# PimLb/POMDP_PBVI_Exploration

Hardware: AMD Instinct MI355X
Metric: alpha-vector backups/sec (higher is better)
Workload: dtype f32

## Files before the change

### include/pbvi_hip.h

```cpp
#ifndef PBVI_HIP_H
#define PBVI_HIP_H

#include <stddef.h>
#include <stdint.h>

#ifdef __cplusplus
extern "C" {
#endif

typedef struct pbvi_engine pbvi_engine_t;

enum pbvi_status {
    PBVI_OK = 0,
    PBVI_EINVAL = -1,
    PBVI_ENOMEM = -2,
    PBVI_ERUNTIME = -3,
    PBVI_EUNSUPPORTED = -4
};

enum pbvi_dtype { PBVI_F32 = 0, PBVI_F64 = 1 };

enum pbvi_mode {
    PBVI_SPARSE = 0,
    PBVI_DENSE = 1
};

enum pbvi_flags {
    PBVI_BELIEF_DOMINANCE = 1
};

typedef struct pbvi_stats {
    double ms_total;
    double ms_project;
    double ms_score;
    double ms_argmax;
    double ms_refine;
    double ms_action;
    double ms_assemble;
    double ms_dominance;
    int64_t n_pairs;
    int64_t n_dead;
    int64_t n_refined;
    int64_t n_refined_actions;
    int64_t n_unique;
    int64_t score_flops;
    int64_t score_flops_executed;
    int64_t score_tiles_dense;
    int64_t score_tiles_run;
    int64_t project_flops;
    int64_t project_flops_executed;
    int32_t split_k;
    int32_t formulation;
    int64_t n_refine_candidates;
    double ms_project_gemm;
    int32_t screened;
    int32_t fused_projection;
    int32_t score_split;
    int32_t gamma_chunks;
} pbvi_stats_t;

int pbvi_version(void);
int pbvi_device_count(void);
const char* pbvi_last_error(void);

int pbvi_engine_create(pbvi_engine_t** out, int device, int32_t S, int32_t A, int32_t O, int32_t R,
                       const int32_t* reach_states, const void* rto, const void* exp_reward,
                       int dtype, int mode);
void pbvi_engine_destroy(pbvi_engine_t* e);

int pbvi_alpha_set(pbvi_engine_t* e, const void* alpha, int64_t V);
int pbvi_alpha_append(pbvi_engine_t* e, const void* alpha, int64_t V_add);
int64_t pbvi_alpha_count(const pbvi_engine_t* e);

int pbvi_beliefs_set(pbvi_engine_t* e, const void* beliefs, int64_t B);

int64_t pbvi_alpha_store_append(pbvi_engine_t* e, const void* rows , int64_t n);
int pbvi_alpha_select(pbvi_engine_t* e, const int32_t* ids , int64_t V);
int pbvi_alpha_layout(pbvi_engine_t* e, int64_t* free_rows, int64_t* layouts);
int pbvi_alpha_store_reset(pbvi_engine_t* e);
int64_t pbvi_belief_store_append(pbvi_engine_t* e, const void* rows , int64_t n);
int pbvi_beliefs_select(pbvi_engine_t* e, const int32_t* ids , int64_t B);
int pbvi_belief_store_reset(pbvi_engine_t* e);

int pbvi_backup_run(pbvi_engine_t* e, double gamma, int flags, pbvi_stats_t* stats );

int pbvi_backup_fetch(pbvi_engine_t* e, void* out_alpha, int32_t* out_action,
                      int32_t* out_best_alpha, uint8_t* out_keep);

int64_t pbvi_backup_unique_count(const pbvi_engine_t* e);
int pbvi_backup_fetch_unique(pbvi_engine_t* e, void* out_rows, int32_t* out_index);

int pbvi_backup_fetch_compact(pbvi_engine_t* e, void* out_rows, int32_t* out_index, int32_t* out_action,
                              int32_t* out_best_alpha, uint8_t* out_keep);

int pbvi_backup_run_fetch(pbvi_engine_t* e, double gamma, int flags, pbvi_stats_t* stats, void* out_rows, int64_t cap_rows,
                          int32_t* out_slot, int32_t* out_index, int32_t* out_action, int32_t* out_best_alpha, uint8_t* out_keep,
                          int64_t* n_unique, int64_t* n_slots);

int pbvi_backup_fetch_row_hashes(pbvi_engine_t* e, uint64_t* out_hashes);

void* pbvi_host_alloc(size_t bytes);
void pbvi_host_free(void* p);

int64_t pbvi_backup_store_unique(pbvi_engine_t* e, const int32_t* unique_idx, int64_t n);

int pbvi_backup_fetch_unique_keys(pbvi_engine_t* e, int32_t* out_keys);
int pbvi_backup_fetch_exchange(pbvi_engine_t* e, int32_t* out);
int pbvi_backup_fetch_exchange_padded(pbvi_engine_t* e, int64_t per, int32_t* out);
int pbvi_assemble_rows(pbvi_engine_t* e, double gamma, int64_t n, const int32_t* keys, void* out_rows);
int64_t pbvi_assemble_rows_store(pbvi_engine_t* e, double gamma, int64_t n, const int32_t* keys, void* out_rows);
int64_t pbvi_exchange_merge(const int32_t* all_meta, int32_t world, int64_t stride, int64_t per, int32_t key_width,
                            int64_t n_total, int32_t* out_keys, int32_t* out_index, int32_t* out_action, uint8_t* out_keep);

int pbvi_backup_device_results(pbvi_engine_t* e, void** d_alpha, int32_t** d_action, uint8_t** d_keep);

int pbvi_backup(pbvi_engine_t* e, const void* beliefs, int64_t B, double gamma, int flags,
                void* out_alpha, int32_t* out_action, int32_t* out_best_alpha, uint8_t* out_keep,
                pbvi_stats_t* stats);

int pbvi_prune_dominated(pbvi_engine_t* e, uint8_t* keep );

int pbvi_value_max(pbvi_engine_t* e, double* out_value, int32_t* out_index);

int pbvi_value_max_store(pbvi_engine_t* e, int64_t n, double* out_value, int32_t* out_index);
int pbvi_backup_fetch_value_max(pbvi_engine_t* e, double* out_value);
int64_t pbvi_belief_store_count(const pbvi_engine_t* e);
int64_t pbvi_alpha_store_count(const pbvi_engine_t* e);

int pbvi_set_value_max_exact(pbvi_engine_t* e, int exact);

int pbvi_belief_update(pbvi_engine_t* e, const int32_t* actions, const int32_t* observations, void* out_beliefs);

int pbvi_beliefs_advance(pbvi_engine_t* e, const int32_t* actions, const int32_t* observations, const uint8_t* keep,
                         int64_t* out_B);
int pbvi_beliefs_fetch(pbvi_engine_t* e, void* out_beliefs);
int64_t pbvi_beliefs_count(const pbvi_engine_t* e);

int pbvi_mdp_value_iteration(int device, int32_t S, int32_t A, int32_t R, const int32_t* reach_states,
                             const double* reach_prob, const double* exp_reward, const double* v0, double gamma,
                             double max_change_limit, int32_t horizon, double* out_rows, double* out_changes,
                             int32_t* out_iterations);

int64_t pbvi_belief_walk(pbvi_engine_t* e, const double* b0, int64_t n, const int32_t* actions, const int32_t* observations,
                         const uint8_t* restart, double* out_beliefs);
int pbvi_belief_walk_keys(pbvi_engine_t* e, int64_t n, uint64_t* out_keys);
int pbvi_engine_set_rto_f64(pbvi_engine_t* e, const double* rto);

int pbvi_set_formulation(pbvi_engine_t* e, int formulation);

int pbvi_set_f64_screen(pbvi_engine_t* e, int mode);

int pbvi_set_fused_projection(pbvi_engine_t* e, int enable);

int pbvi_set_score_split(pbvi_engine_t* e, int mode);

int pbvi_set_gamma_tiling(pbvi_engine_t* e, int mode, int64_t chunk_rows);
int pbvi_gamma_tiling_plan(int32_t S, int32_t A, int32_t O, int64_t V, int64_t B, int dtype, int64_t budget_bytes,
                           int64_t* chunk_rows, int64_t* n_chunks, int64_t* bytes_needed);

int pbvi_set_tie_window(pbvi_engine_t* e, double rel);

int pbvi_debug_poison(int enable);
int64_t pbvi_debug_alloc_limit(int64_t mb);
int pbvi_engine_after_oom(pbvi_engine_t* e);

int pbvi_debug_gemm_dense(int enable);

int64_t pbvi_device_bytes(const pbvi_engine_t* e);

#ifdef __cplusplus
}
#endif
#endif
```

### pomdp_pbvi_exploration_amd/csrc/engine.hip

```cpp
#include <algorithm>
#include <cmath>
#include <cstdio>
#include <cstdlib>
#include <cstring>
#include <condition_variable>
#include <mutex>
#include <new>
#include <string>
#include <thread>
#include <unistd.h>
#include <vector>

#include "backup_kernels.h"
#include "split_bf16.h"

namespace pbvi {

static thread_local std::string g_err;
static int g_poison = -1;
static bool poison_enabled() {
    if (g_poison < 0) g_poison = getenv("PBVI_POISON") != nullptr ? 1 : 0;
    return g_poison == 1;
}
void set_error(const std::string& msg) { g_err = msg; }
// ... 3523 lines not shown
    do {                                                   \
        if (!(e) || !(e)->impl) {                          \
            pbvi::set_error("NULL engine handle");         \
            return PBVI_EINVAL;                            \
        }                                                  \
    } while (0)

int pbvi_alpha_set(pbvi_engine_t* e, const void* alpha, int64_t V) {
    NEED(e);
    return e->impl->alpha_set(alpha, V);
}
int pbvi_alpha_append(pbvi_engine_t* e, const void* alpha, int64_t V_add) {
    NEED(e);
    return e->impl->alpha_append(alpha, V_add);
}
int64_t pbvi_alpha_count(const pbvi_engine_t* e) { return (e && e->impl) ? e->impl->alpha_count() : -1; }
int pbvi_beliefs_set(pbvi_engine_t* e, const void* beliefs, int64_t B) {
    NEED(e);
    return e->impl->beliefs_set(beliefs, B);
}
int pbvi_backup_run(pbvi_engine_t* e, double gamma, int flags, pbvi_stats_t* stats) {
    NEED(e);
    return e->impl->backup_run(gamma, flags, stats);
}
int pbvi_backup_fetch(pbvi_engine_t* e, void* out_alpha, int32_t* out_action, int32_t* out_best_alpha, uint8_t* out_keep) {
    NEED(e);
    return e->impl->backup_fetch(out_alpha, out_action, out_best_alpha, out_keep);
}
int64_t pbvi_backup_store_unique(pbvi_engine_t* e, const int32_t* unique_idx, int64_t n) {
    NEED(e);
    return e->impl->store_append_unique(unique_idx, n);
}

int pbvi_backup_fetch_row_hashes(pbvi_engine_t* e, uint64_t* out_hashes) {
    NEED(e);
    return e->impl->fetch_row_hashes(out_hashes);
}
int pbvi_backup_fetch_unique_keys(pbvi_engine_t* e, int32_t* out_keys) {
    NEED(e);
    return e->impl->fetch_unique_keys(out_keys);
}
int pbvi_backup_fetch_exchange(pbvi_engine_t* e, int32_t* out) {
    NEED(e);
    return e->impl->fetch_exchange(out, e->impl->beliefs_count());
}
int pbvi_backup_fetch_exchange_padded(pbvi_engine_t* e, int64_t per, int32_t* out) {
    NEED(e);
    return e->impl->fetch_exchange(out, per);
}
int64_t pbvi_assemble_rows_store(pbvi_engine_t* e, double gamma, int64_t n, const int32_t* keys, void* out_rows) {
    NEED(e);
    return e->impl->assemble_keys_store(gamma, n, keys, out_rows);
}
int64_t pbvi_exchange_merge(const int32_t* all_meta, int32_t world, int64_t stride, int64_t per, int32_t key_width,
                            int64_t n_total, int32_t* out_keys, int32_t* out_index, int32_t* out_action, uint8_t* out_keep) {
    if (!all_meta || world <= 0 || per <= 0 || key_width <= 0 || n_total < 0 || !out_keys || !out_index ||
        !out_action || !out_keep) {
        pbvi::set_error("exchange_merge: bad arguments");
        return PBVI_EINVAL;
    }
    const int64_t n_meta = 1 + 3 * per + per * (int64_t)key_width;
    if (per > 0x7fffffff / ((int64_t)key_width + 3) || stride < n_meta || n_total > (int64_t)world * per ||
        (int64_t)world * per > 0x7fffffff) {
        pbvi::set_error("exchange_merge: message stride / belief count do not fit the block size");
        return PBVI_EINVAL;
    }
    int64_t total = 0;
    for (int r = 0; r < world; ++r) {
        const int64_t c = all_meta[(int64_t)r * stride];
        if (c < 0 || c > per) {
            pbvi::set_error("exchange_merge: corrupt message (unique-row count out of range)");
            return PBVI_EINVAL;
        }
        total += c;
    }
    size_t cap = 16;
    while (cap < (size_t)total * 2 + 1) cap <<= 1;
    std::vector<int32_t> table, pos;
    try {
        table.assign(cap, -1);
        pos.assign((size_t)std::max<int64_t>(total, 1), 0);
    } catch (const std::bad_alloc&) {
        pbvi::set_error("exchange_merge: host allocation failed");
        return PBVI_ENOMEM;
    }
    int64_t n_keys = 0, base = 0;
    for (int r = 0; r < world; ++r) {
        const int32_t* msg = all_meta + (int64_t)r * stride;
        const int32_t* keys = msg + 1 + 3 * per;
        const int64_t c = msg[0];
        for (int64_t u = 0; u < c; ++u) {
            const int32_t* k = keys + u * key_width;
            uint64_t h = 1469598103934665603ull;
            for (int j = 0; j < key_width; ++j) h = (h ^ (uint32_t)k[j]) * 1099511628211ull;
            size_t slot = (size_t)(h ^ (h >> 29)) & (cap - 1);
            for (;;) {
                const int32_t at = table[slot];
                if (at < 0) {
                    std::memcpy(out_keys + n_keys * key_width, k, (size_t)key_width * sizeof(int32_t));
                    table[slot] = (int32_t)n_keys;
                    pos[(size_t)(base + u)] = (int32_t)n_keys++;
                    break;
                }
                if (std::memcmp(out_keys + (int64_t)at * key_width, k, (size_t)key_width * sizeof(int32_t)) == 0) {
                    pos[(size_t)(base + u)] = at;
                    break;
                }
                slot = (slot + 1) & (cap - 1);
            }
        }
        const int64_t lo = std::min<int64_t>((int64_t)r * per, n_total), hi = std::min<int64_t>(lo + per, n_total);
        for (int64_t j = 0; j < hi - lo; ++j) {
            const int32_t u = msg[1 + j];
            if (u < 0 || u >= c) {
                pbvi::set_error("exchange_merge: corrupt message (row index out of range)");
                return PBVI_EINVAL;
            }
            out_index[lo + j] = pos[(size_t)(base + u)];
            out_action[lo + j] = msg[1 + per + j];
            out_keep[lo + j] = msg[1 + 2 * per + j] ? 1 : 0;
        }
        base += c;
    }
    return n_keys;
}
int pbvi_assemble_rows(pbvi_engine_t* e, double gamma, int64_t n, const int32_t* keys, void* out_rows) {
    NEED(e);
    return e->impl->assemble_keys(gamma, n, keys, out_rows);
}
int pbvi_engine_after_oom(pbvi_engine_t* e) {
    NEED(e);
    return e->impl->after_oom();
}
int pbvi_backup_device_results(pbvi_engine_t* e, void** d_alpha, int32_t** d_action, uint8_t** d_keep) {
    NEED(e);
    return e->impl->device_results(d_alpha, d_action, d_keep);
}
int64_t pbvi_backup_unique_count(const pbvi_engine_t* e) { return (e && e->impl) ? e->impl->unique_count() : -1; }
int pbvi_backup_fetch_unique(pbvi_engine_t* e, void* out_rows, int32_t* out_index) {
    NEED(e);
    return e->impl->fetch_unique(out_rows, out_index);
}
int pbvi_backup_run_fetch(pbvi_engine_t* e, double gamma, int flags, pbvi_stats_t* stats, void* out_rows, int64_t cap_rows,
                          int32_t* out_slot, int32_t* out_index, int32_t* out_action, int32_t* out_best_alpha, uint8_t* out_keep,
                          int64_t* n_unique, int64_t* n_slots) {
    NEED(e);
    return e->impl->run_fetch(gamma, flags, stats, out_rows, cap_rows, out_slot, out_index, out_action, out_best_alpha, out_keep,
                              n_unique, n_slots);
}
int pbvi_backup_fetch_compact(pbvi_engine_t* e, void* out_rows, int32_t* out_index, int32_t* out_action,
                              int32_t* out_best_alpha, uint8_t* out_keep) {
    NEED(e);
    return e->impl->fetch_compact(out_rows, out_index, out_action, out_best_alpha, out_keep);
}
void* pbvi_host_alloc(size_t bytes) {
    void* p = nullptr;
    if (bytes == 0) return nullptr;
    if (hipHostMalloc(&p, bytes, hipHostMallocDefault) != hipSuccess) {
        (void)hipGetLastError();
        pbvi::set_error("pbvi_host_alloc: hipHostMalloc of " + std::to_string(bytes) + " bytes failed");
        return nullptr;
    }
    return p;
}
void pbvi_host_free(void* p) {
    if (p && hipHostFree(p) != hipSuccess) (void)hipGetLastError();
}
int pbvi_debug_gemm_dense(int enable) { return pbvi::set_gemm_force_dense(enable); }
int pbvi_backup(pbvi_engine_t* e, const void* beliefs, int64_t B, double gamma, int flags, void* out_alpha,
                int32_t* out_action, int32_t* out_best_alpha, uint8_t* out_keep, pbvi_stats_t* stats) {
    NEED(e);
    int rc = e->impl->beliefs_set(beliefs, B);
    if (rc) return rc;
    rc = e->impl->backup_run(gamma, flags, stats);
    if (rc) return rc;
    return e->impl->backup_fetch(out_alpha, out_action, out_best_alpha, out_keep);
}
int pbvi_prune_dominated(pbvi_engine_t* e, uint8_t* keep) {
    NEED(e);
    return e->impl->prune_dominated(keep);
}
int pbvi_value_max(pbvi_engine_t* e, double* out_value, int32_t* out_index) {
    NEED(e);
    return e->impl->value_max(out_value, out_index);
}
int64_t pbvi_alpha_store_append(pbvi_engine_t* e, const void* rows, int64_t n) {
    NEED(e);
    return e->impl->store_append(0, rows, n);
}
int pbvi_value_max_store(pbvi_engine_t* e, int64_t n, double* out_value, int32_t* out_index) {
    NEED(e);
    return e->impl->value_max_store(n, out_value, out_index);
}
int64_t pbvi_belief_store_count(const pbvi_engine_t* e) { return (e && e->impl) ? e->impl->store_count(1) : -1; }
int64_t pbvi_alpha_store_count(const pbvi_engine_t* e) { return (e && e->impl) ? e->impl->store_count(0) : -1; }
int pbvi_alpha_select(pbvi_engine_t* e, const int32_t* ids, int64_t V) {
    NEED(e);
    return e->impl->store_select(0, ids, V);
}
int pbvi_alpha_store_reset(pbvi_engine_t* e) {
    NEED(e);
    return e->impl->store_reset(0);
}
int64_t pbvi_belief_store_append(pbvi_engine_t* e, const void* rows, int64_t n) {
    NEED(e);
    return e->impl->store_append(1, rows, n);
}
int pbvi_beliefs_select(pbvi_engine_t* e, const int32_t* ids, int64_t B) {
    NEED(e);
    return e->impl->store_select(1, ids, B);
}
int pbvi_belief_store_reset(pbvi_engine_t* e) {
    NEED(e);
    return e->impl->store_reset(1);
}
int pbvi_beliefs_advance(pbvi_engine_t* e, const int32_t* actions, const int32_t* observations, const uint8_t* keep,
                         int64_t* out_B) {
    NEED(e);
    return e->impl->beliefs_advance(actions, observations, keep, out_B);
}

int pbvi_backup_fetch_value_max(pbvi_engine_t* e, double* out_value) {
    NEED(e);
    return e->impl->backup_value_max(out_value);
}
int pbvi_belief_walk_keys(pbvi_engine_t* e, int64_t n, uint64_t* out_keys) {
    NEED(e);
    return e->impl->walk_keys(n, out_keys);
}
int64_t pbvi_belief_walk(pbvi_engine_t* e, const double* b0, int64_t n, const int32_t* actions, const int32_t* observations,
                         const uint8_t* restart, double* out_beliefs) {
    NEED(e);
    return e->impl->belief_walk(b0, n, actions, observations, restart, out_beliefs);
}

int pbvi_engine_set_rto_f64(pbvi_engine_t* e, const double* rto) {
    NEED(e);
    return e->impl->set_rto_f64(rto);
}

int pbvi_beliefs_fetch(pbvi_engine_t* e, void* out_beliefs) {
    NEED(e);
    return e->impl->beliefs_fetch(out_beliefs);
}

int64_t pbvi_beliefs_count(const pbvi_engine_t* e) { return (e && e->impl) ? e->impl->beliefs_count() : -1; }

int pbvi_mdp_value_iteration(int device, int32_t S, int32_t A, int32_t R, const int32_t* reach_states,
                             const double* reach_prob, const double* exp_reward, const double* v0, double gamma,
                             double max_change_limit, int32_t horizon, double* out_rows, double* out_changes,
                             int32_t* out_iterations) {
    return pbvi::mdp_value_iteration(device, S, A, R, reach_states, reach_prob, exp_reward, v0, gamma, max_change_limit,
                                     horizon, out_rows, out_changes, out_iterations);
}

int pbvi_belief_update(pbvi_engine_t* e, const int32_t* actions, const int32_t* observations, void* out_beliefs) {
    NEED(e);
    return e->impl->belief_update(actions, observations, out_beliefs);
}
int pbvi_set_formulation(pbvi_engine_t* e, int formulation) {
    NEED(e);
    return e->impl->set_formulation(formulation);
}
int pbvi_set_fused_projection(pbvi_engine_t* e, int enable) {
    NEED(e);
    return e->impl->set_fused(enable);
}
int pbvi_set_f64_screen(pbvi_engine_t* e, int mode) {
    NEED(e);
    return e->impl->set_screen(mode);
}
int pbvi_set_score_split(pbvi_engine_t* e, int mode) {
    NEED(e);
    return e->impl->set_score_split(mode);
}
int pbvi_set_value_max_exact(pbvi_engine_t* e, int exact) {
    NEED(e);
    return e->impl->set_value_max_exact(exact);
}
int pbvi_alpha_layout(pbvi_engine_t* e, int64_t* free_rows, int64_t* layouts) {
    NEED(e);
    return e->impl->alpha_layout(free_rows, layouts);
}
int pbvi_set_gamma_tiling(pbvi_engine_t* e, int mode, int64_t chunk_rows) {
    NEED(e);
    return e->impl->set_gamma_tiling(mode, chunk_rows);
}
int pbvi_gamma_tiling_plan(int32_t S, int32_t A, int32_t O, int64_t V, int64_t B, int dtype, int64_t budget_bytes,
                           int64_t* chunk_rows, int64_t* n_chunks, int64_t* bytes_needed) {
    using namespace pbvi;
    if (!chunk_rows || !n_chunks || !bytes_needed || (dtype != 0 && dtype != 1))
        FAIL(PBVI_EINVAL, "gamma_tiling_plan: null output or dtype not 0 (fp32) / 1 (fp64)");
    pbvi::TilingPlan tp;
    const int rc = pbvi::tiling_plan(S, A, O, V, B, dtype == 0, budget_bytes, *chunk_rows, &tp);
    if (rc == PBVI_EINVAL) FAIL(PBVI_EINVAL, "gamma_tiling_plan: S, A, O, V, B must be positive, budget and chunk_rows >= 0, A*O*(V+1)+2A within int32");
    *chunk_rows = tp.chunk_rows;
    *n_chunks = tp.n_chunks;
    *bytes_needed = tp.bytes;
    if (rc == PBVI_ENOMEM)
        FAIL(PBVI_ENOMEM, "gamma_tiling_plan: chunks of " + std::to_string(tp.chunk_rows) + " alpha rows need " +
                              std::to_string(tp.bytes) + " bytes, the budget is " + std::to_string(budget_bytes));
    return PBVI_OK;
}
int pbvi_set_tie_window(pbvi_engine_t* e, double rel) {
    NEED(e);
    return e->impl->set_tie_window(rel);
}
int64_t pbvi_device_bytes(const pbvi_engine_t* e) { return (e && e->impl) ? e->impl->device_bytes() : -1; }

}
```

### pomdp_pbvi_exploration_amd/csrc/gemm.hip

```cpp
#include "pbvi_common.h"
#include "split_bf16.h"

#include <cstdlib>
#include <map>
#include <mutex>

namespace pbvi {

typedef float f32x4 __attribute__((ext_vector_type(4)));
typedef float f32x16 __attribute__((ext_vector_type(16)));

constexpr int TILE_FLOATS = 256 * GEMM_BK;
constexpr int KL_IRR_BIT = 30;
constexpr int KL_MASK = (1 << KL_IRR_BIT) - 1;
constexpr int GEMM_LDS_BYTES = 4 * TILE_FLOATS * 4;

__device__ __forceinline__ void glds16(const float* g, float* l) {
    __builtin_amdgcn_global_load_lds((const __attribute__((address_space(1))) void*)g,
                                     (__attribute__((address_space(3))) void*)l, 16, 0, 0);
}

struct TileThread {
    int lane, wid, i, h, wr, wc;
    int srow[4], scol[4];
    int a_row[4], b_row[2];
    __device__ __forceinline__ void init() {
        const int tid = threadIdx.x;
        lane = tid & 63;
        wid = __builtin_amdgcn_readfirstlane(tid >> 6);
        i = lane & 31;
        h = lane >> 5;
        wr = wid >> 2;
        wc = wid & 3;
#pragma unroll
        for (int it = 0; it < 4; ++it) {
            const int c = it * 512 + tid;
            const int row = c >> 3, pc = c & 7;
            srow[it] = row;
            scol[it] = (pc ^ ((row >> 1) & 7)) * 4;
        }
#pragma unroll
        for (int mi = 0; mi < 4; ++mi) a_row[mi] = wr * 128 + mi * 32 + i;
#pragma unroll
        for (int ni = 0; ni < 2; ++ni) b_row[ni] = wc * 64 + ni * 32 + i;
    }
};

__device__ __forceinline__ void tile_stage(const TileThread& t, float* lds, int buf, const float* Ablk, int lda,
                                           const float* Bblk, int ldb, int kt) {
    float* la = lds + buf * 2 * TILE_FLOATS;
    float* lb = la + TILE_FLOATS;
#pragma unroll
    for (int it = 0; it < 4; ++it) {
        const int wave_chunk = it * 512 + t.wid * 64;
        glds16(Ablk + (int64_t)t.srow[it] * lda + kt * GEMM_BK + t.scol[it], la + wave_chunk * 4);
        glds16(Bblk + (int64_t)t.srow[it] * ldb + kt * GEMM_BK + t.scol[it], lb + wave_chunk * 4);
    }
}

__device__ __forceinline__ void tile_compute_group(const TileThread& t, const float* lds, int buf, f32x16 (&acc)[4][2], int g) {
    const float* la = lds + buf * 2 * TILE_FLOATS;
    const float* lb = la + TILE_FLOATS;
    f32x4 af[4], bf[2];
#pragma unroll
    for (int mi = 0; mi < 4; ++mi) {
        const int pc = (2 * g + t.h) ^ ((t.a_row[mi] >> 1) & 7);
        af[mi] = *(const f32x4*)(la + t.a_row[mi] * GEMM_BK + pc * 4);
    }
#pragma unroll
    for (int ni = 0; ni < 2; ++ni) {
        const int pc = (2 * g + t.h) ^ ((t.b_row[ni] >> 1) & 7);
        bf[ni] = *(const f32x4*)(lb + t.b_row[ni] * GEMM_BK + pc * 4);
    }
#pragma unroll
    for (int j = 0; j < 4; ++j)
#pragma unroll
        for (int mi = 0; mi < 4; ++mi)
#pragma unroll
            for (int ni = 0; ni < 2; ++ni)
                acc[mi][ni] = __builtin_amdgcn_mfma_f32_32x32x2f32(af[mi][j], bf[ni][j], acc[mi][ni], 0, 0, 0);
}

__device__ __forceinline__ void tile_compute(const TileThread& t, const float* lds, int buf, f32x16 (&acc)[4][2]) {
#pragma unroll
    for (int g = 0; g < 4; ++g) tile_compute_group(t, lds, buf, acc, g);
}

__device__ __forceinline__ void tile_run(const TileThread& t, float* lds, const float* Ablk, int lda, const float* Bblk,
                                         int ldb, const int* __restrict__ kl, int i0, int i1, f32x16 (&acc)[4][2]) {
    tile_stage(t, lds, 0, Ablk, lda, Bblk, ldb, kl[i0] & KL_MASK);
    int k_next = (i0 + 1 < i1) ? (kl[i0 + 1] & KL_MASK) : 0;
    asm volatile("s_waitcnt vmcnt(0)" ::: "memory");
    __syncthreads();
    int buf = 0;
    for (int it = i0; it < i1; ++it) {
        int k_after = 0;
        if (it + 1 < i1) {
            tile_stage(t, lds, buf ^ 1, Ablk, lda, Bblk, ldb, k_next);
            if (it + 2 < i1) k_after = kl[it + 2] & KL_MASK;
        }
        tile_compute(t, lds, buf, acc);
        asm volatile("s_waitcnt vmcnt(0)" ::: "memory");
        __syncthreads();
        buf ^= 1;
        k_next = k_after;
    }
}

__device__ __forceinline__ void tile_zero(f32x16 (&acc)[4][2]) {
#pragma unroll
    for (int mi = 0; mi < 4; ++mi)
#pragma unroll
        for (int ni = 0; ni < 2; ++ni)
#pragma unroll
            for (int e = 0; e < 16; ++e) acc[mi][ni][e] = 0.f;
}

__device__ __forceinline__ void tile_store(const TileThread& t, float* Cz, int ldc, int tm, int tn,
                                           const f32x16 (&acc)[4][2]) {
#pragma unroll
    for (int mi = 0; mi < 4; ++mi)
#pragma unroll
        for (int ni = 0; ni < 2; ++ni) {
            const int col = tn * 256 + t.wc * 64 + ni * 32 + t.i;
#pragma unroll
            for (int e = 0; e < 16; ++e) {
                const int row = tm * 256 + t.wr * 128 + mi * 32 + (e & 3) + 8 * (e >> 2) + 4 * t.h;
                Cz[(int64_t)row * ldc + col] = acc[mi][ni][e];
            }
        }
}

__global__ __launch_bounds__(512) void k_gemm_nt_f32_mfma(
    const float* __restrict__ A, int lda, const float* __restrict__ B, int ldb, float* __restrict__ C,
    int ldc, int64_t slab_stride, int tiles_m, int tiles_n, int k_tiles, int chunk_len, int max_chunks,
    const int* __restrict__ klist, const int* __restrict__ kcount, int64_t batch_stride_b, int64_t batch_stride_c) {
    extern __shared__ __attribute__((aligned(16))) float lds[];
    const int bid = blockIdx.x;
    const int xcd = bid & 7, slot = bid >> 3;
    const int tm = slot % tiles_m;
    const int q = (slot / tiles_m) * 8 + xcd;
    const int tn = q % tiles_n;
    const int z = q / tiles_n;
    if (z >= max_chunks) return;
    const int batch = blockIdx.y;
    B += batch * batch_stride_b;
    C += batch * batch_stride_c;
    const int pair = (batch * tiles_n + tn) * tiles_m + tm;
    const int cnt = kcount[pair];
    const int i0 = z * chunk_len;
    const int i1 = (i0 + chunk_len < cnt) ? i0 + chunk_len : cnt;
    if (i0 >= i1) return;
    TileThread t;
    t.init();
    f32x16 acc[4][2];
    tile_zero(acc);
    tile_run(t, lds, A + (int64_t)tm * 256 * lda, lda, B + (int64_t)tn * 256 * ldb, ldb,
             klist + (int64_t)pair * k_tiles, i0, i1, acc);
    tile_store(t, C + (int64_t)z * slab_stride, ldc, tm, tn, acc);
}

__global__ void k_streamk_plan(const int* __restrict__ kcount, int pairs, int nblocks, int k_tiles, int max_split,
                               int ovh, int* __restrict__ prefix, int* __restrict__ start_pair,
                               int* __restrict__ first_block, int* __restrict__ nchunks, int* __restrict__ plan) {
    __shared__ int part[256];
    __shared__ int q_sh;
    const int tid = threadIdx.x;
    const int per = (pairs + 255) / 256;
    const int p0 = (tid * per < pairs) ? tid * per : pairs;
    const int p1 = (p0 + per < pairs) ? p0 + per : pairs;
    int sum = 0;
    for (int p = p0; p < p1; ++p) {
        const int cnt = kcount[p];
        sum += cnt > 0 ? cnt + ovh : 0;
    }
    part[tid] = sum;
    for (int i = tid; i < nblocks; i += 256) start_pair[i] = -1;
    __syncthreads();
    if (tid == 0) {
        int run = 0;
        for (int i = 0; i < 256; ++i) {
            const int v = part[i];
            part[i] = run;
            run += v;
        }
        int q = (run + nblocks - 1) / nblocks;
        const int qmin = (k_tiles + ovh + max_split - 1) / max_split;
        if (q < qmin) q = qmin;
        if (q < 1) q = 1;
        q_sh = q;
        plan[0] = q;
        plan[1] = run;
        prefix[pairs] = run;
    }
    __syncthreads();
    const int q = q_sh;
    int run = part[tid];
    for (int p = p0; p < p1; ++p) {
        const int cnt = kcount[p];
        prefix[p] = run;
        if (cnt > 0) {
            const int cost = cnt + ovh;
            const int fb = run / q, lb = (run + cost - 1) / q;
            const int fw = (run + ovh) / q;
            first_block[p] = fw;
            nchunks[p] = lb - fw + 1;
            for (int i = fb; i <= lb; ++i)
                if ((int64_t)i * q >= run) start_pair[i] = p;
            run += cost;
        } else {
            first_block[p] = 0;
            nchunks[p] = 0;
        }
    }
}

__global__ __launch_bounds__(512) void k_gemm_nt_f32_streamk(
    const float* __restrict__ A, int lda, const float* __restrict__ B, int ldb, float* __restrict__ C, int ldc,
    int64_t slab_stride, int tiles_m, int pairs, int k_tiles, const int* __restrict__ klist,
    const int* __restrict__ kcount, const int* __restrict__ prefix, const int* __restrict__ start_pair,
    const int* __restrict__ first_block, const int* __restrict__ plan, int ovh) {
    extern __shared__ __attribute__((aligned(16))) float lds[];
    const int nb = gridDim.x;
    int L;
    {
        const int bid = blockIdx.x, xcd = bid & 7, qq = nb >> 3, r = nb & 7;
        const int base = (xcd < r) ? xcd * (qq + 1) : r * (qq + 1) + (xcd - r) * qq;
        L = base + (bid >> 3);
    }
    const int q = plan[0], T = plan[1];
    int64_t pos = (int64_t)L * q;
    if (pos >= T) return;
    const int64_t end = (pos + q < T) ? pos + q : T;
    int p = start_pair[L];
    if (p < 0) return;
    TileThread t;
    t.init();
    while (pos < end && p < pairs) {
        const int cnt = kcount[p];
        if (cnt == 0) {
            ++p;
            continue;
        }
        const int u_lo = (int)(pos - prefix[p]);
        const int64_t room = end - pos;
        const int u_hi = (u_lo + room < cnt + ovh) ? (int)(u_lo + room) : cnt + ovh;
        const int lo = u_lo > ovh ? u_lo - ovh : 0;
        const int hi = u_hi > ovh ? u_hi - ovh : 0;
        if (hi > lo) {
            const int tm = p % tiles_m, tn = p / tiles_m;
            f32x16 acc[4][2];
            tile_zero(acc);
            tile_run(t, lds, A + (int64_t)tm * 256 * lda, lda, B + (int64_t)tn * 256 * ldb, ldb,
                     klist + (int64_t)p * k_tiles, lo, hi, acc);
            const bool cont = L != first_block[p];
            tile_store(t, cont ? C + slab_stride + (int64_t)L * (256 * 256) : C, cont ? 256 : ldc, cont ? 0 : tm, cont ? 0 : tn, acc);
        }
        pos += u_hi - u_lo;
        ++p;
    }
}

typedef int i32x4 __attribute__((ext_vector_type(4)));
#ifndef PBVI_FUSED_EXP
#define PBVI_FUSED_EXP 0
#endif

__device__ __forceinline__ void ld16(f32x4& dst, const float* p) {
    asm volatile("global_load_dwordx4 %0, %1, off" : "=v"(dst) : "v"(p) : "memory");
}
__device__ __forceinline__ void ld16i(i32x4& dst, const int32_t* p) {
    asm volatile("global_load_dwordx4 %0, %1, off" : "=v"(dst) : "v"(p) : "memory");
}
__device__ __forceinline__ void ld4(float& dst, const float* p) {
    asm volatile("global_load_dword %0, %1, off" : "=v"(dst) : "v"(p) : "memory");
}

__device__ __forceinline__ f32x4 fused_value(float gamma, f32x4 w, f32x4 av) {
#pragma clang fp contract(off)
    const f32x4 pr = w * av;
    return gamma * pr;
}

__device__ __forceinline__ void tile_run_fused(const TileThread& t, float* lds, const float* Ablk, int lda,
                                               const int32_t* __restrict__ rsrow, const float* __restrict__ rtorow,
                                               const float* __restrict__ arow0, int64_t a_step ,
                                               float gamma, const int* __restrict__ kl,
                                               int i0, int i1, f32x16 (&acc)[4][2]) {
    const int tid = threadIdx.x;
    auto stage_a = [&](int buf, int entry) {
        const int kt = entry & KL_MASK;
        float* la = lds + buf * 2 * TILE_FLOATS;
#pragma unroll
        for (int it = 0; it < 4; ++it)
            glds16(Ablk + (int64_t)t.srow[it] * lda + kt * GEMM_BK + t.scol[it], la + (it * 512 + t.wid * 64) * 4);
    };
    i32x4 idx;
    f32x4 w, av[4];
    auto tables = [&](int entry) {
        const int s = (entry & KL_MASK) * GEMM_BK + t.scol[0];
        ld16i(idx, rsrow + s);
        ld16(w, rtorow + s);
    };
    auto alphas = [&](int entry) {
        if (entry >> KL_IRR_BIT) {
#pragma unroll
            for (int it = 0; it < 4; ++it) {
                const float* arow = arow0 + it * a_step;
                float e0, e1, e2, e3;
                ld4(e0, arow + idx[0]);
                ld4(e1, arow + idx[1]);
                ld4(e2, arow + idx[2]);
                ld4(e3, arow + idx[3]);
                asm volatile("s_waitcnt vmcnt(0)\n\tv_mov_b32 %0, %4\n\tv_mov_b32 %1, %5\n\tv_mov_b32 %2, %6\n\tv_mov_b32 %3, %7"
                             : "=&v"(av[it].x), "=&v"(av[it].y), "=&v"(av[it].z), "=&v"(av[it].w)
                             : "v"(e0), "v"(e1), "v"(e2), "v"(e3)
                             : "memory");
            }
        } else {
#if PBVI_FUSED_EXP == 1
#pragma unroll
            for (int it = 0; it < 4; ++it) av[it] = w;
#else
#pragma unroll
            for (int it = 0; it < 4; ++it) ld16(av[it], arow0 + it * a_step + idx[0]);
#endif
        }
    };
    auto store_b = [&](int buf) {
        float* lb = lds + buf * 2 * TILE_FLOATS + TILE_FLOATS;
#if PBVI_FUSED_EXP == 2
        if (gamma == 12345.f)
#endif
#pragma unroll
        for (int it = 0; it < 4; ++it) *(f32x4*)(lb + (it * 512 + tid) * 4) = fused_value(gamma, w, av[it]);
    };
    tables(kl[i0]);
    stage_a(0, kl[i0]);
    asm volatile("s_waitcnt vmcnt(0)" : "+v"(idx), "+v"(w)::"memory");
    alphas(kl[i0]);
    asm volatile("s_waitcnt vmcnt(0)" : "+v"(av[0]), "+v"(av[1]), "+v"(av[2]), "+v"(av[3])::"memory");
    store_b(0);
    int k_next = (i0 + 1 < i1) ? kl[i0 + 1] : 0;
    __syncthreads();
    int buf = 0;
    for (int it = i0; it < i1; ++it) {
        int k_after = 0;
        const bool more = it + 1 < i1;
        if (more) {
            tables(k_next);
            stage_a(buf ^ 1, k_next);
            if (it + 2 < i1) k_after = kl[it + 2];
        }
        tile_compute_group(t, lds, buf, acc, 0);
        if (more) {
            asm volatile("s_waitcnt vmcnt(4)" : "+v"(idx), "+v"(w)::"memory");
            alphas(k_next);
        }
        tile_compute_group(t, lds, buf, acc, 1);
        tile_compute_group(t, lds, buf, acc, 2);
        if (more) {
            asm volatile("s_waitcnt vmcnt(0)" : "+v"(av[0]), "+v"(av[1]), "+v"(av[2]), "+v"(av[3])::"memory");
            store_b(buf ^ 1);
        }
        tile_compute_group(t, lds, buf, acc, 3);
        asm volatile("s_waitcnt vmcnt(0)" ::: "memory");
        __syncthreads();
        buf ^= 1;
        k_next = k_after;
    }
}

__global__ __launch_bounds__(512) void k_gemm_nt_f32_streamk_fused(
    const float* __restrict__ A, int lda, const float* __restrict__ B, int ldb, FusedB fb, float* __restrict__ C, int ldc,
    int64_t slab_stride, int tiles_m, int pairs, int k_tiles, const int* __restrict__ klist, const int* __restrict__ kcount,
    const int* __restrict__ prefix, const int* __restrict__ start_pair, const int* __restrict__ first_block,
    const int* __restrict__ plan, int ovh) {
    extern __shared__ __attribute__((aligned(16))) float lds[];
    const int nb = gridDim.x;
    int L;
    {
        const int bid = blockIdx.x, xcd = bid & 7, qq = nb >> 3, r = nb & 7;
        const int base = (xcd < r) ? xcd * (qq + 1) : r * (qq + 1) + (xcd - r) * qq;
        L = base + (bid >> 3);
    }
    const int q = plan[0], T = plan[1];
    int64_t pos = (int64_t)L * q;
    if (pos >= T) return;
    const int64_t end = (pos + q < T) ? pos + q : T;
    int p = start_pair[L];
    if (p < 0) return;
    TileThread t;
    t.init();
    while (pos < end && p < pairs) {
        const int cnt = kcount[p];
        if (cnt == 0) {
            ++p;
            continue;
        }
        const int u_lo = (int)(pos - prefix[p]);
        const int64_t room = end - pos;
        const int u_hi = (u_lo + room < cnt + ovh) ? (int)(u_lo + room) : cnt + ovh;
        const int lo = u_lo > ovh ? u_lo - ovh : 0;
        const int hi = u_hi > ovh ? u_hi - ovh : 0;
        if (hi > lo) {
            const int tm = p % tiles_m, tn = p / tiles_m;
            f32x16 acc[4][2];
            tile_zero(acc);
            if (fb.mat[tn]) {
                const int bt = fb.ctile != nullptr ? fb.ctile[tn] : tn;
                tile_run(t, lds, A + (int64_t)tm * 256 * lda, lda, B + (int64_t)bt * 256 * ldb, ldb,
                         klist + (int64_t)p * k_tiles, lo, hi, acc);
            } else {
                const int r0 = tn * 256;
                const int g = r0 / fb.V, v0 = r0 - g * fb.V;
                tile_run_fused(t, lds, A + (int64_t)tm * 256 * lda, lda, fb.rs + (int64_t)(g / fb.O) * fb.S_pad,
                               fb.rto + (int64_t)g * fb.S_pad, fb.alpha + (int64_t)(v0 + t.srow[0]) * fb.lda,
                               (int64_t)64 * fb.lda, fb.gamma,
                               klist + (int64_t)p * k_tiles, lo, hi, acc);
            }
            const bool cont = L != first_block[p];
            tile_store(t, cont ? C + slab_stride + (int64_t)L * (256 * 256) : C, cont ? 256 : ldc, cont ? 0 : tm, cont ? 0 : tn, acc);
        }
        pos += u_hi - u_lo;
        ++p;
    }
}

constexpr int FUSED_R_MAX = 7;
constexpr int TAB_WORDS = 8 * GEMM_BK;
constexpr int GEMM_LDS_BYTES_R = GEMM_LDS_BYTES + 2 * 2 * TAB_WORDS * 4;

struct Frag {
    f32x4 af[4], bf[2];
};
__device__ __forceinline__ void frag_load(const TileThread& t, const float* lds, int buf, int g, Frag& f) {
    const float* la = lds + buf * 2 * TILE_FLOATS;
    const float* lb = la + TILE_FLOATS;
#pragma unroll
    for (int mi = 0; mi < 4; ++mi) {
        const int pc = (2 * g + t.h) ^ ((t.a_row[mi] >> 1) & 7);
        f.af[mi] = *(const f32x4*)(la + t.a_row[mi] * GEMM_BK + pc * 4);
    }
#pragma unroll
    for (int ni = 0; ni < 2; ++ni) {
        const int pc = (2 * g + t.h) ^ ((t.b_row[ni] >> 1) & 7);
        f.bf[ni] = *(const f32x4*)(lb + t.b_row[ni] * GEMM_BK + pc * 4);
    }
}
__device__ __forceinline__ void frag_mfma(const Frag& f, int j, f32x16 (&acc)[4][2]) {
#pragma unroll
    for (int mi = 0; mi < 4; ++mi)
#pragma unroll
        for (int ni = 0; ni < 2; ++ni)
            acc[mi][ni] = __builtin_amdgcn_mfma_f32_32x32x2f32(f.af[mi][j], f.bf[ni][j], acc[mi][ni], 0, 0, 0);
}

__device__ __forceinline__ f32x4 proj_add(f32x4 acc, f32x4 w, f32x4 av) {
#pragma clang fp contract(off)
    const f32x4 pr = w * av;
    return acc + pr;
}
__device__ __forceinline__ f32x4 proj_scale(float gamma, f32x4 acc) {
#pragma clang fp contract(off)
    return gamma * acc;
}

template <int R>
__device__ __forceinline__ void tile_run_fused_r(const TileThread& t, float* lds, const float* Ablk, int lda,
                                                 const float* Bblk, int ldb, const int32_t* __restrict__ rs_a,
                                                 const float* __restrict__ rto_g, int S_pad,
                                                 const float* __restrict__ arow0, int64_t a_step ,
                                                 float gamma, const int* __restrict__ kl, int i0, int i1,
                                                 f32x16 (&acc)[4][2]) {
    const int tid = threadIdx.x;
    int32_t* tabi = (int32_t*)(lds + 4 * TILE_FLOATS);
    float* tabw = (float*)(tabi + 2 * TAB_WORDS);
    constexpr int nunits = 2 * R;
    static_assert(R >= 2 && R <= FUSED_R_MAX, "2R + 2 issue points must fit the 16 of a K step");
    const int scol0 = t.scol[0];
    auto stage_a = [&](int buf, int entry) {
        const int kt = entry & KL_MASK;
        float* la = lds + buf * 2 * TILE_FLOATS;
#pragma unroll
        for (int it = 0; it < 4; ++it)
            glds16(Ablk + (int64_t)t.srow[it] * lda + kt * GEMM_BK + t.scol[it], la + (it * 512 + t.wid * 64) * 4);
    };
    auto stage_b = [&](int buf, int entry) {
        const int kt = entry & KL_MASK;
        float* lb = lds + buf * 2 * TILE_FLOATS + TILE_FLOATS;
#pragma unroll
        for (int it = 0; it < 4; ++it)
            glds16(Bblk + (int64_t)t.srow[it] * ldb + kt * GEMM_BK + t.scol[it], lb + (it * 512 + t.wid * 64) * 4);
    };
    auto stage_tab = [&](int tb, int entry) {
        if (t.wid == 0 && t.lane < 8 * R) {
            const int64_t off = (int64_t)(t.lane >> 3) * S_pad + (entry & KL_MASK) * GEMM_BK + (t.lane & 7) * 4;
            glds16((const float*)(rs_a + off), (float*)(tabi + tb * TAB_WORDS));
            glds16(rto_g + off, tabw + tb * TAB_WORDS);
        }
    };
    f32x4 av[2][2];
    f32x4 pacc[2];
    auto unit_issue = [&](int u, int slot, int tb) {
        const int hh = u >= R ? 1 : 0, r = u - hh * R;
        const i32x4 idx = *(const i32x4*)(tabi + tb * TAB_WORDS + r * GEMM_BK + scol0);
#if PBVI_FUSED_EXP == 3
        const float* p0 = arow0 + (int64_t)(2 * hh) * a_step + (idx[0] & 3);
#else
        const float* p0 = arow0 + (int64_t)(2 * hh) * a_step + idx[0];
#endif
        ld16(av[slot][0], p0);
        ld16(av[slot][1], p0 + a_step);
    };
    auto unit_consume = [&](int u, int slot, int tb, int dst_buf, bool last_in_queue) {
        const int hh = u >= R ? 1 : 0, r = u - hh * R;
        const f32x4 w = *(const f32x4*)(tabw + tb * TAB_WORDS + r * GEMM_BK + scol0);
        if (last_in_queue)
            asm volatile("s_waitcnt vmcnt(0)" : "+v"(av[slot][0]), "+v"(av[slot][1])::"memory");
        else
            asm volatile("s_waitcnt vmcnt(2)" : "+v"(av[slot][0]), "+v"(av[slot][1])::"memory");
        if (r == 0) {
            pacc[0] = f32x4{0.f, 0.f, 0.f, 0.f};
            pacc[1] = f32x4{0.f, 0.f, 0.f, 0.f};
        }
        pacc[0] = proj_add(pacc[0], w, av[slot][0]);
        pacc[1] = proj_add(pacc[1], w, av[slot][1]);
        if (r == R - 1) {
            float* lb = lds + dst_buf * 2 * TILE_FLOATS + TILE_FLOATS;
            *(f32x4*)(lb + ((2 * hh) * 512 + tid) * 4) = proj_scale(gamma, pacc[0]);
            *(f32x4*)(lb + ((2 * hh + 1) * 512 + tid) * 4) = proj_scale(gamma, pacc[1]);
        }
    };
    {
        const int e0 = kl[i0];
        stage_a(0, e0);
        if (e0 >> KL_IRR_BIT) {
            stage_b(0, e0);
        } else {
            stage_tab(0, e0);
            asm volatile("s_waitcnt vmcnt(0)" ::: "memory");
            __syncthreads();
            for (int u = 0; u < nunits; ++u) {
                unit_issue(u, 0, 0);
                unit_consume(u, 0, 0, 0, true);
            }
        }
    }
    int e_next = (i0 + 1 < i1) ? kl[i0 + 1] : 0;
    if (i0 + 1 < i1 && !(e_next >> KL_IRR_BIT)) stage_tab(1, e_next);
    int e_after = (i0 + 2 < i1) ? kl[i0 + 2] : 0;
    asm volatile("s_waitcnt vmcnt(0)" ::: "memory");
    __syncthreads();
    int buf = 0;
    for (int it = i0; it < i1; ++it) {
        const bool more = it + 1 < i1;
        const bool gen = more && !(e_next >> KL_IRR_BIT);
        int e_after2 = 0;
        if (more) {
            stage_a(buf ^ 1, e_next);
            if (!gen) stage_b(buf ^ 1, e_next);
            if (it + 2 < i1 && !(e_after >> KL_IRR_BIT)) stage_tab(buf, e_after);
            if (it + 3 < i1) e_after2 = kl[it + 3];
        }
        Frag f;
#pragma unroll
        for (int g = 0; g < 4; ++g) {
            frag_load(t, lds, buf, g, f);
#pragma unroll
            for (int j = 0; j < 4; ++j) {
                const int p = 4 * g + j;
                if (gen) {
                    if (p >= 2 && p - 2 < nunits) unit_consume(p - 2, p & 1, buf ^ 1, buf ^ 1, p - 2 == nunits - 1);
                    if (p < nunits) unit_issue(p, p & 1, buf ^ 1);
                }
                frag_mfma(f, j, acc);
            }
        }
        asm volatile("s_waitcnt vmcnt(0)" ::: "memory");
        __syncthreads();
        buf ^= 1;
        e_next = e_after;
        e_after = e_after2;
    }
}

template <int R>
__global__ __launch_bounds__(512) void k_gemm_nt_f32_streamk_fused_r(
    const float* __restrict__ A, int lda, const float* __restrict__ B, int ldb, FusedB fb, float* __restrict__ C, int ldc,
    int64_t slab_stride, int tiles_m, int pairs, int k_tiles, const int* __restrict__ klist, const int* __restrict__ kcount,
    const int* __restrict__ prefix, const int* __restrict__ start_pair, const int* __restrict__ first_block,
    const int* __restrict__ plan, int ovh) {
    extern __shared__ __attribute__((aligned(16))) float lds[];
    const int nb = gridDim.x;
    int L;
    {
        const int bid = blockIdx.x, xcd = bid & 7, qq = nb >> 3, r = nb & 7;
        const int base = (xcd < r) ? xcd * (qq + 1) : r * (qq + 1) + (xcd - r) * qq;
        L = base + (bid >> 3);
    }
    const int q = plan[0], T = plan[1];
    int64_t pos = (int64_t)L * q;
    if (pos >= T) return;
    const int64_t end = (pos + q < T) ? pos + q : T;
    int p = start_pair[L];
    if (p < 0) return;
    TileThread t;
    t.init();
    while (pos < end && p < pairs) {
        const int cnt = kcount[p];
        if (cnt == 0) {
            ++p;
            continue;
        }
        const int u_lo = (int)(pos - prefix[p]);
        const int64_t room = end - pos;
        const int u_hi = (u_lo + room < cnt + ovh) ? (int)(u_lo + room) : cnt + ovh;
        const int lo = u_lo > ovh ? u_lo - ovh : 0;
        const int hi = u_hi > ovh ? u_hi - ovh : 0;
        if (hi > lo) {
            const int tm = p % tiles_m, tn = p / tiles_m;
            f32x16 acc[4][2];
            tile_zero(acc);
            if (fb.mat[tn]) {
                tile_run(t, lds, A + (int64_t)tm * 256 * lda, lda, B + (int64_t)tn * 256 * ldb, ldb,
                         klist + (int64_t)p * k_tiles, lo, hi, acc);
            } else {
                const int r0 = tn * 256;
                const int g = r0 / fb.V, v0 = r0 - g * fb.V;
                tile_run_fused_r<R>(t, lds, A + (int64_t)tm * 256 * lda, lda, B + (int64_t)tn * 256 * ldb, ldb,
                                 fb.rs + (int64_t)(g / fb.O) * R * fb.S_pad, fb.rto + (int64_t)g * R * fb.S_pad,
                                 fb.S_pad, fb.alpha + (int64_t)(v0 + t.srow[0]) * fb.lda, (int64_t)64 * fb.lda, fb.gamma,
                                 klist + (int64_t)p * k_tiles, lo, hi, acc);
            }
            const bool cont = L != first_block[p];
            tile_store(t, cont ? C + slab_stride + (int64_t)L * (256 * 256) : C, cont ? 256 : ldc, cont ? 0 : tm, cont ? 0 : tn, acc);
        }
        pos += u_hi - u_lo;
        ++p;
    }
}

typedef __bf16 bf16x8 __attribute__((ext_vector_type(8)));

__device__ __forceinline__ void split_store(float* lop, int row, int kg, const f32x4& x0, const f32x4& x1) {
    i32x4 hi, lo;
    uint32_t h, l;
    split_pair(x0[0], x0[1], h, l); hi[0] = (int)h; lo[0] = (int)l;
    split_pair(x0[2], x0[3], h, l); hi[1] = (int)h; lo[1] = (int)l;
    split_pair(x1[0], x1[1], h, l); hi[2] = (int)h; lo[2] = (int)l;
    split_pair(x1[2], x1[3], h, l); hi[3] = (int)h; lo[3] = (int)l;
    const int sw = (row >> 1) & 7;
    *(i32x4*)(lop + row * GEMM_BK + (kg ^ sw) * 4) = hi;
    *(i32x4*)(lop + row * GEMM_BK + ((4 + kg) ^ sw) * 4) = lo;
}

struct SplitFrag {
    i32x4 ah[4], al[4], bh[2], bl[2];
};
__device__ __forceinline__ void split_group(const TileThread& t, const float* lds, int buf, int kk, int term, SplitFrag& f,
                                            f32x16 (&acc)[4][2]) {
    const float* la = lds + buf * 2 * TILE_FLOATS;
    const float* lb = la + TILE_FLOATS;
    const int hc = 2 * kk + t.h;
    if (term != 1) {
#pragma unroll
        for (int mi = 0; mi < 4; ++mi) {
            const int r = t.a_row[mi], sw = (r >> 1) & 7;
            if (term == 0) f.ah[mi] = *(const i32x4*)(la + r * GEMM_BK + (hc ^ sw) * 4);
            else f.al[mi] = *(const i32x4*)(la + r * GEMM_BK + ((4 + hc) ^ sw) * 4);
        }
    }
    if (term != 2) {
#pragma unroll
        for (int ni = 0; ni < 2; ++ni) {
            const int r = t.b_row[ni], sw = (r >> 1) & 7;
            if (term == 0) f.bh[ni] = *(const i32x4*)(lb + r * GEMM_BK + (hc ^ sw) * 4);
            else f.bl[ni] = *(const i32x4*)(lb + r * GEMM_BK + ((4 + hc) ^ sw) * 4);
        }
    }
#pragma unroll
    for (int mi = 0; mi < 4; ++mi)
#pragma unroll
        for (int ni = 0; ni < 2; ++ni) {
            const i32x4 a = term == 2 ? f.al[mi] : f.ah[mi];
            const i32x4 b = term == 1 ? f.bl[ni] : f.bh[ni];
            acc[mi][ni] = __builtin_amdgcn_mfma_f32_32x32x16_bf16(__builtin_bit_cast(bf16x8, a), __builtin_bit_cast(bf16x8, b),
                                                                  acc[mi][ni], 0, 0, 0);
        }
}

__device__ __forceinline__ void tile_run_split(const TileThread& t, float* lds, const float* Aplane, int lda, const float* Bblk,
                                               int ldb, bool gen, const int32_t* __restrict__ rsrow,
                                               const float* __restrict__ rtorow, const float* __restrict__ arow0,
                                               int64_t a_step, float gamma, const int* __restrict__ kl, int i0, int i1,
                                               f32x16 (&acc)[4][2]) {
    const int tid = threadIdx.x;
    const int kg = tid & 3, r0 = tid >> 2;
    f32x4 xb[2][2];
    i32x4 idx[2];
    f32x4 w[2];
    const uint32_t a_off = (uint32_t)(t.srow[0] * lda + t.scol[0]) * 4u;
    auto stage_a = [&](int buf, int entry) {
        const char* base = (const char*)(Aplane + (int64_t)(entry & KL_MASK) * GEMM_BK);
        float* la = lds + buf * 2 * TILE_FLOATS;
#pragma unroll
        for (int it = 0; it < 4; ++it)
            glds16((const float*)(base + (int64_t)it * 64 * lda * 4 + a_off), la + (it * 512 + t.wid * 64) * 4);
    };
    auto load_rows = [&](int entry) {
        const int k = (entry & KL_MASK) * GEMM_BK + kg * 8;
#pragma unroll
        for (int it = 0; it < 2; ++it) {
            const float* p = Bblk + (int64_t)(it * 128 + r0) * ldb + k;
            ld16(xb[it][0], p);
            ld16(xb[it][1], p + 4);
        }
    };
    auto indices = [&](int entry) {
        const int s = (entry & KL_MASK) * GEMM_BK + kg * 8;
        ld16i(idx[0], rsrow + s);
        ld16i(idx[1], rsrow + s + 4);
    };
    auto weights = [&](int entry) {
        const int s = (entry & KL_MASK) * GEMM_BK + kg * 8;
        ld16(w[0], rtorow + s);
        ld16(w[1], rtorow + s + 4);
    };
    auto alphas = [&](int entry) {
        if (entry >> KL_IRR_BIT) {
#pragma unroll
            for (int it = 0; it < 2; ++it) {
                const float* arow = arow0 + it * a_step;
#pragma unroll
                for (int q = 0; q < 2; ++q) {
                    float e0, e1, e2, e3;
                    ld4(e0, arow + idx[q][0]);
                    ld4(e1, arow + idx[q][1]);
                    ld4(e2, arow + idx[q][2]);
                    ld4(e3, arow + idx[q][3]);
                    asm volatile("s_waitcnt vmcnt(0)\n\tv_mov_b32 %0, %4\n\tv_mov_b32 %1, %5\n\tv_mov_b32 %2, %6\n\tv_mov_b32 %3, %7"
                                 : "=&v"(xb[it][q].x), "=&v"(xb[it][q].y), "=&v"(xb[it][q].z), "=&v"(xb[it][q].w)
                                 : "v"(e0), "v"(e1), "v"(e2), "v"(e3)
                                 : "memory");
                }
            }
        } else {
#pragma unroll
            for (int it = 0; it < 2; ++it) {
                ld16(xb[it][0], arow0 + it * a_step + idx[0][0]);
                ld16(xb[it][1], arow0 + it * a_step + idx[1][0]);
            }
        }
    };
    auto store_b = [&](int buf, int it) {
        float* lb = lds + buf * 2 * TILE_FLOATS + TILE_FLOATS;
        if (gen)
            split_store(lb, it * 128 + r0, kg, fused_value(gamma, w[0], xb[it][0]), fused_value(gamma, w[1], xb[it][1]));
        else
            split_store(lb, it * 128 + r0, kg, xb[it][0], xb[it][1]);
    };
    {
        const int e0 = kl[i0];
        if (gen) {
            indices(e0);
            weights(e0);
            asm volatile("s_waitcnt vmcnt(0)" : "+v"(idx[0]), "+v"(idx[1])::"memory");
            alphas(e0);
            indices(i0 + 1 < i1 ? kl[i0 + 1] : 0);
        } else {
            load_rows(e0);
        }
        stage_a(0, e0);
        asm volatile("s_waitcnt vmcnt(0)" : "+v"(xb[0][0]), "+v"(xb[0][1]), "+v"(xb[1][0]), "+v"(xb[1][1]), "+v"(w[0]), "+v"(w[1]),
                     "+v"(idx[0]), "+v"(idx[1])::"memory");
        store_b(0, 0);
        store_b(0, 1);
    }
    int k_next = (i0 + 1 < i1) ? kl[i0 + 1] : 0;
    int k_after = (i0 + 2 < i1) ? kl[i0 + 2] : 0;
    __syncthreads();
    int buf = 0;
    for (int it = i0; it < i1; ++it) {
        int k_after2 = 0;
        const bool more = it + 1 < i1;
        if (more) {
            if (gen) {
                alphas(k_next);
                weights(k_next);
                indices(k_after);
            } else {
                load_rows(k_next);
            }
            stage_a(buf ^ 1, k_next);
            if (it + 3 < i1) k_after2 = kl[it + 3];
        }
        SplitFrag f;
        split_group(t, lds, buf, 0, 0, f, acc);
        split_group(t, lds, buf, 0, 1, f, acc);
        split_group(t, lds, buf, 0, 2, f, acc);
        split_group(t, lds, buf, 1, 0, f, acc);
        if (more) {
            if (gen)
                asm volatile("s_waitcnt vmcnt(6)" : "+v"(xb[0][0]), "+v"(xb[0][1]), "+v"(xb[1][0]), "+v"(xb[1][1]), "+v"(w[0]),
                             "+v"(w[1])::"memory");
            else
                asm volatile("s_waitcnt vmcnt(4)" : "+v"(xb[0][0]), "+v"(xb[0][1]), "+v"(xb[1][0]), "+v"(xb[1][1])::"memory");
            store_b(buf ^ 1, 0);
        }
        split_group(t, lds, buf, 1, 1, f, acc);
        if (more) store_b(buf ^ 1, 1);
        split_group(t, lds, buf, 1, 2, f, acc);
        asm volatile("s_waitcnt vmcnt(0)" : "+v"(idx[0]), "+v"(idx[1])::"memory");
        __syncthreads();
        buf ^= 1;
        k_next = k_after;
        k_after = k_after2;
    }
}

__global__ __launch_bounds__(512) void k_gemm_split_streamk(
    const float* __restrict__ A, int lda, const float* __restrict__ B, int ldb, FusedB fb, float* __restrict__ C, int ldc,
    int64_t slab_stride, int tiles_m, int pairs, int k_tiles, const int* __restrict__ klist, const int* __restrict__ kcount,
    const int* __restrict__ prefix, const int* __restrict__ start_pair, const int* __restrict__ first_block,
    const int* __restrict__ plan, int ovh) {
    extern __shared__ __attribute__((aligned(16))) float lds[];
    const int nb = gridDim.x;
    int L;
    {
        const int bid = blockIdx.x, xcd = bid & 7, qq = nb >> 3, r = nb & 7;
        const int base = (xcd < r) ? xcd * (qq + 1) : r * (qq + 1) + (xcd - r) * qq;
        L = base + (bid >> 3);
    }
    const int q = plan[0], T = plan[1];
    int64_t pos = (int64_t)L * q;
    if (pos >= T) return;
    const int64_t end = (pos + q < T) ? pos + q : T;
    int p = start_pair[L];
    if (p < 0) return;
    TileThread t;
    t.init();
    while (pos < end && p < pairs) {
        const int cnt = kcount[p];
        if (cnt == 0) {
            ++p;
            continue;
        }
        const int u_lo = (int)(pos - prefix[p]);
        const int64_t room = end - pos;
        const int u_hi = (u_lo + room < cnt + ovh) ? (int)(u_lo + room) : cnt + ovh;
        const int lo = u_lo > ovh ? u_lo - ovh : 0;
        const int hi = u_hi > ovh ? u_hi - ovh : 0;
        if (hi > lo) {
            const int tm = p % tiles_m, tn = p / tiles_m;
            f32x16 acc[4][2];
            tile_zero(acc);
            const float* Ablk = A + (int64_t)tm * 256 * lda;
            if (fb.mat == nullptr || fb.mat[tn]) {
                const int bt = (fb.mat != nullptr && fb.ctile != nullptr) ? fb.ctile[tn] : tn;
                tile_run_split(t, lds, Ablk, lda, B + (int64_t)bt * 256 * ldb, ldb, false, nullptr, nullptr, nullptr, 0, 0.f,
                               klist + (int64_t)p * k_tiles, lo, hi, acc);
            } else {
                const int r0 = tn * 256;
                const int g = r0 / fb.V, v0 = r0 - g * fb.V;
                tile_run_split(t, lds, Ablk, lda, nullptr, 0, true, fb.rs + (int64_t)(g / fb.O) * fb.S_pad,
                               fb.rto + (int64_t)g * fb.S_pad, fb.alpha + (int64_t)(v0 + (threadIdx.x >> 2)) * fb.lda,
                               (int64_t)128 * fb.lda, fb.gamma, klist + (int64_t)p * k_tiles, lo, hi, acc);
            }
            const bool cont = L != first_block[p];
            tile_store(t, cont ? C + slab_stride + (int64_t)L * (256 * 256) : C, cont ? 256 : ldc, cont ? 0 : tm, cont ? 0 : tn, acc);
        }
        pos += u_hi - u_lo;
        ++p;
    }
}

__global__ void k_split_probe(float* out) {
    const int lane = threadIdx.x, r = lane & 31, h = lane >> 5;
    float a[8] = {0.f, 0.f, 0.f, 0.f, 0.f, 0.f, 0.f, 0.f}, b[8] = {0.f, 0.f, 0.f, 0.f, 0.f, 0.f, 0.f, 0.f};
    const float x = 0x1.02p-120f + 0x1p-132f;
    if (h == 0) {
        a[0] = x;
        a[1] = 0x1p-100f;
        if (r == 0) b[0] = 1.f;
        if (r == 1) b[1] = 0x1p-30f;
    }
    i32x4 ah, al, bh, bl;
    uint32_t hh, ll;
#pragma unroll
    for (int p = 0; p < 4; ++p) {
        split_pair(a[2 * p], a[2 * p + 1], hh, ll); ah[p] = (int)hh; al[p] = (int)ll;
        split_pair(b[2 * p], b[2 * p + 1], hh, ll); bh[p] = (int)hh; bl[p] = (int)ll;
    }
    f32x16 acc;
#pragma unroll
    for (int e = 0; e < 16; ++e) acc[e] = 0.f;
    acc = __builtin_amdgcn_mfma_f32_32x32x16_bf16(__builtin_bit_cast(bf16x8, ah), __builtin_bit_cast(bf16x8, bh), acc, 0, 0, 0);
    acc = __builtin_amdgcn_mfma_f32_32x32x16_bf16(__builtin_bit_cast(bf16x8, ah), __builtin_bit_cast(bf16x8, bl), acc, 0, 0, 0);
    acc = __builtin_amdgcn_mfma_f32_32x32x16_bf16(__builtin_bit_cast(bf16x8, al), __builtin_bit_cast(bf16x8, bh), acc, 0, 0, 0);
    if (lane < 2) out[lane] = acc[0];
    if (lane == 0) out[2] = x;
}

int gemm_split_supported(int device) {
    static std::mutex mu;
    static std::map<int, int> known;
    std::lock_guard<std::mutex> lock(mu);
    auto it = known.find(device);
    if (it != known.end()) return it->second;
    int ok = 0;
    float* d = nullptr;
    hipStream_t st = nullptr;
    float h[3] = {0.f, 0.f, 0.f};
    if (hipStreamCreateWithFlags(&st, hipStreamNonBlocking) == hipSuccess && hipMalloc((void**)&d, sizeof(h)) == hipSuccess) {
        hipLaunchKernelGGL(k_split_probe, dim3(1), dim3(64), 0, st, d);
        if (hipGetLastError() == hipSuccess && hipMemcpyAsync(h, d, sizeof(h), hipMemcpyDeviceToHost, st) == hipSuccess &&
            hipStreamSynchronize(st) == hipSuccess)
            ok = (h[0] == h[2] && h[1] == 0x1p-130f) ? 1 : 0;
    }
    (void)hipGetLastError();
    if (d != nullptr) (void)hipFree(d);
    if (st != nullptr) (void)hipStreamDestroy(st);
    known[device] = ok;
    return ok;
}

__global__ void k_tile_nonzero(const float* __restrict__ X, int ld, int k_tiles, uint8_t* __restrict__ nz) {
    const int tile = blockIdx.y;
    const int row = tile * 256 + threadIdx.x;
    const f32x4* p = (const f32x4*)(X + (int64_t)row * ld);
    for (int j = 0; j < 8; ++j) {
        const int kt = blockIdx.x * 8 + j;
        if (kt >= k_tiles) break;
        int f = 0;
#pragma unroll
        for (int c = 0; c < 8; ++c) {
            const f32x4 v = p[kt * 8 + c];
            f |= (v[0] != 0.f) | (v[1] != 0.f) | (v[2] != 0.f) | (v[3] != 0.f);
        }
        const int any = __syncthreads_or(f);
        if (threadIdx.x == 0) nz[(int64_t)tile * k_tiles + kt] = any ? 1 : 0;
    }
}

__global__ void k_build_klists(const uint8_t* __restrict__ nzA, const uint8_t* __restrict__ nzB, int G,
                               int v_group, int n_rows, int tiles_m, int k_tiles, int chunk_len, int force_dense,
                               int* __restrict__ klist, int* __restrict__ kcount, int* __restrict__ nchunks,
                               const int32_t* __restrict__ irr, int groups_per_action) {
    __shared__ int wcount[4];
    __shared__ int total;
    const int tiles_n = gridDim.x / tiles_m;
    const int batch = blockIdx.y;
    const int tm = blockIdx.x % tiles_m, tn = blockIdx.x / tiles_m;
    const int pair = (batch * tiles_n + tn) * tiles_m + tm;
    const int tid = threadIdx.x, lane = tid & 63, wid = tid >> 6;
    const int r0 = tn * 256;
    int r1 = r0 + 255;
    if (r1 >= n_rows) r1 = n_rows - 1;
    int g0 = 0, g1 = -1;
    if (nzB != nullptr && G > 0 && r0 < n_rows) {
        if (r1 >= G * v_group) {
            g0 = 0;
            g1 = G;
        } else {
            g0 = r0 / v_group;
            g1 = r1 / v_group;
        }
    }
    if (tid == 0) total = 0;
    __syncthreads();
    for (int base = 0; base < k_tiles; base += 256) {
        const int kt = base + tid;
        int f = 0;
        if (force_dense) {
            f = kt < k_tiles;
        } else if (kt < k_tiles && r0 < n_rows && nzA[(int64_t)tm * k_tiles + kt]) {
            if (nzB == nullptr) {
                f = 1;
            } else if (G == 0) {
                f = nzB[((int64_t)batch * tiles_n + tn) * k_tiles + kt];
            } else {
                for (int g = g0; g <= g1; ++g) f |= nzB[(int64_t)g * k_tiles + kt];
            }
        }
        const unsigned long long mask = __ballot(f);
        if (lane == 0) wcount[wid] = __popcll(mask);
        __syncthreads();
        int off = total;
        for (int w = 0; w < wid; ++w) off += wcount[w];
        if (f) {
            int entry = kt;
            if (irr != nullptr && g0 == g1 && g1 < G && irr[(int64_t)(g0 / groups_per_action) * k_tiles + kt]) entry |= 1 << KL_IRR_BIT;
            klist[(int64_t)pair * k_tiles + off + __popcll(mask & ((1ull << lane) - 1ull))] = entry;
        }
        __syncthreads();
        if (tid == 0) total += wcount[0] + wcount[1] + wcount[2] + wcount[3];
        __syncthreads();
    }
    if (tid == 0) {
        kcount[pair] = total;
        nchunks[pair] = (total + chunk_len - 1) / chunk_len;
    }
}

static int g_force_dense = -1;
int gemm_force_dense() {
    if (g_force_dense < 0) g_force_dense = getenv("PBVI_GEMM_DENSE") ? (atoi(getenv("PBVI_GEMM_DENSE")) != 0) : 0;
    return g_force_dense;
}
int set_gemm_force_dense(int enable) {
    const int prev = gemm_force_dense();
    g_force_dense = enable ? 1 : 0;
    return prev;
}

int choose_chunk_len(int tiles_mn, int k_tiles) {
    if (const char* env = getenv("PBVI_GEMM_CHUNK")) {
        const int v = atoi(env);
        if (v > 0) return v < k_tiles ? v : k_tiles;
    }
    const int64_t total = (int64_t)tiles_mn * k_tiles;
    int64_t len = total / (256 * 8);
    if (len < 8) len = 8;
    if (len > 96) len = 96;
    if (len > k_tiles) len = k_tiles;
    return (int)len;
}

static int device_cu_count() {
    static int cus = 0;
    if (cus == 0) {
        int dev = 0;
        hipDeviceProp_t prop;
        if (hipGetDevice(&dev) == hipSuccess && hipGetDeviceProperties(&prop, dev) == hipSuccess)
            cus = prop.multiProcessorCount;
        if (cus <= 0) cus = 256;
    }
    return cus;
}

hipError_t launch_tile_nonzero_f32(const float* X, int ld, int rows_pad, int k_tiles, uint8_t* nz, hipStream_t stream) {
    dim3 grid((k_tiles + 7) / 8, rows_pad / 256);
    hipLaunchKernelGGL(k_tile_nonzero, grid, dim3(256), 0, stream, X, ld, k_tiles, nz);
    return hipGetLastError();
}

static hipError_t set_lds_attr() {
    static bool done = false;
    if (done) return hipSuccess;
    hipError_t e = hipFuncSetAttribute((const void*)k_gemm_nt_f32_mfma, hipFuncAttributeMaxDynamicSharedMemorySize,
                                       GEMM_LDS_BYTES);
    if (e != hipSuccess) return e;
    e = hipFuncSetAttribute((const void*)k_gemm_nt_f32_streamk, hipFuncAttributeMaxDynamicSharedMemorySize,
                            GEMM_LDS_BYTES);
    if (e != hipSuccess) return e;
    e = hipFuncSetAttribute((const void*)k_gemm_nt_f32_streamk_fused, hipFuncAttributeMaxDynamicSharedMemorySize,
                            GEMM_LDS_BYTES);
    if (e != hipSuccess) return e;
    e = hipFuncSetAttribute((const void*)k_gemm_split_streamk, hipFuncAttributeMaxDynamicSharedMemorySize, GEMM_LDS_BYTES);
    if (e != hipSuccess) return e;
#define PBVI_FUSED_R_ATTR(RR)                                                                                          \
    e = hipFuncSetAttribute((const void*)k_gemm_nt_f32_streamk_fused_r<RR>, hipFuncAttributeMaxDynamicSharedMemorySize, \
                            GEMM_LDS_BYTES_R);                                                                          \
    if (e != hipSuccess) return e;
    PBVI_FUSED_R_ATTR(2) PBVI_FUSED_R_ATTR(3) PBVI_FUSED_R_ATTR(4) PBVI_FUSED_R_ATTR(5) PBVI_FUSED_R_ATTR(6) PBVI_FUSED_R_ATTR(7)
#undef PBVI_FUSED_R_ATTR
    done = true;
    return hipSuccess;
}

hipError_t launch_gemm_nt_f32(const float* A, int lda, const float* B, int ldb, float* C, const GemmPlan& pl,
                              const uint8_t* nzA, const uint8_t* nzB, int G, int v_group, int n_rows, int* klist,
                              int* kcount, int* nchunks, hipStream_t stream, int batch, int64_t batch_stride_b,
                              int64_t batch_stride_c, int* streamk_ws, hipStream_t list_stream, hipEvent_t list_event,
                              hipEvent_t ev_before, hipEvent_t ev_after, const FusedB* fused, int split) {
    hipError_t e = set_lds_attr();
    if (e != hipSuccess) return e;
    if (batch < 1 || batch > 65535) return hipErrorInvalidValue;
    const int pairs = pl.tiles_m * pl.tiles_n;
    const int force_dense = gemm_force_dense();
    hipStream_t ls = (list_stream != nullptr && list_event != nullptr) ? list_stream : stream;
    if (fused != nullptr && !pl.streamk) return hipErrorInvalidValue;
    if (split && (!pl.streamk || (fused != nullptr && fused->R != 1))) return hipErrorInvalidValue;
    hipLaunchKernelGGL(k_build_klists, dim3(pairs, batch), dim3(256), 0, ls, nzA, nzB, G, v_group, n_rows,
                       pl.tiles_m, pl.k_tiles, pl.chunk_len, force_dense, klist, kcount, nchunks,
                       fused != nullptr ? fused->irr : nullptr, fused != nullptr ? fused->O : 1);
    e = hipGetLastError();
    if (e != hipSuccess) return e;
    if (pl.streamk) {
        if (batch != 1 || streamk_ws == nullptr) return hipErrorInvalidValue;
        int* prefix = streamk_ws;
        int* start_pair = prefix + pairs + 1;
        int* first_block = start_pair + pl.nblocks;
        int* plan = first_block + pairs;
        static const int ovh = getenv("PBVI_STREAMK_OVH") ? atoi(getenv("PBVI_STREAMK_OVH")) : 1;
        hipLaunchKernelGGL(k_streamk_plan, dim3(1), dim3(256), 0, ls, kcount, pairs, pl.nblocks, pl.k_tiles,
                           pl.max_chunks - 1, ovh, prefix, start_pair, first_block, nchunks, plan);
        e = hipGetLastError();
        if (e != hipSuccess) return e;
        if (ls != stream) {
            if ((e = hipEventRecord(list_event, ls)) != hipSuccess) return e;
            if ((e = hipStreamWaitEvent(stream, list_event, 0)) != hipSuccess) return e;
        }
        if (split) {
            FusedB fb{};
            if (fused != nullptr) fb = *fused;
            hipLaunchKernelGGL(k_gemm_split_streamk, dim3(pl.nblocks), dim3(512), GEMM_LDS_BYTES, stream, A, lda, B, ldb, fb, C,
                               pl.ldc, pl.slab_stride, pl.tiles_m, pairs, pl.k_tiles, klist, kcount, prefix, start_pair,
                               first_block, plan, ovh);
        } else if (fused != nullptr && fused->R > 1) {
            switch (fused->R) {
#define PBVI_FUSED_R_CASE(RR)                                                                                                   \
    case RR:                                                                                                                    \
        hipLaunchKernelGGL(k_gemm_nt_f32_streamk_fused_r<RR>, dim3(pl.nblocks), dim3(512), GEMM_LDS_BYTES_R, stream, A, lda, B, \
                           ldb, *fused, C, pl.ldc, pl.slab_stride, pl.tiles_m, pairs, pl.k_tiles, klist, kcount, prefix,        \
                           start_pair, first_block, plan, ovh);                                                                 \
        break;
                PBVI_FUSED_R_CASE(2) PBVI_FUSED_R_CASE(3) PBVI_FUSED_R_CASE(4) PBVI_FUSED_R_CASE(5) PBVI_FUSED_R_CASE(6) PBVI_FUSED_R_CASE(7)
#undef PBVI_FUSED_R_CASE
                default:
                    return hipErrorInvalidValue;
            }
        } else if (fused != nullptr)
            hipLaunchKernelGGL(k_gemm_nt_f32_streamk_fused, dim3(pl.nblocks), dim3(512), GEMM_LDS_BYTES, stream, A, lda, B, ldb,
                               *fused, C, pl.ldc, pl.slab_stride, pl.tiles_m, pairs, pl.k_tiles, klist, kcount, prefix, start_pair,
                               first_block, plan, ovh);
        else
            hipLaunchKernelGGL(k_gemm_nt_f32_streamk, dim3(pl.nblocks), dim3(512), GEMM_LDS_BYTES, stream, A, lda, B, ldb, C,
                               pl.ldc, pl.slab_stride, pl.tiles_m, pairs, pl.k_tiles, klist, kcount, prefix, start_pair,
                               first_block, plan, ovh);
        return hipGetLastError();
    }
    if (ls != stream) {
        if ((e = hipEventRecord(list_event, ls)) != hipSuccess) return e;
        if ((e = hipStreamWaitEvent(stream, list_event, 0)) != hipSuccess) return e;
    }
    const int64_t groups = ((int64_t)pl.tiles_n * pl.max_chunks + 7) / 8 * 8;
    const int64_t total = groups * pl.tiles_m;
    if (total <= 0 || total > 0x7fffffff) return hipErrorInvalidValue;
    if (ev_before != nullptr && (e = hipEventRecord(ev_before, stream)) != hipSuccess) return e;
    hipLaunchKernelGGL(k_gemm_nt_f32_mfma, dim3((unsigned)total, batch), dim3(512), GEMM_LDS_BYTES, stream, A, lda, B,
                       ldb, C, pl.ldc, pl.slab_stride, pl.tiles_m, pl.tiles_n, pl.k_tiles, pl.chunk_len, pl.max_chunks,
                       klist, kcount, batch_stride_b, batch_stride_c);
    if ((e = hipGetLastError()) != hipSuccess) return e;
    if (ev_after != nullptr && (e = hipEventRecord(ev_after, stream)) != hipSuccess) return e;
    return hipSuccess;
}

GemmPlan make_gemm_plan(int M_pad, int N_pad, int K_pad, bool single_chunk) {
    GemmPlan pl;
    pl.tiles_m = M_pad / GEMM_BM;
    pl.tiles_n = N_pad / GEMM_BN;
    pl.k_tiles = K_pad / GEMM_BK;
    pl.ldc = N_pad;
    pl.slab_stride = (int64_t)M_pad * N_pad;
    static const int no_streamk = getenv("PBVI_GEMM_NO_STREAMK") ? atoi(getenv("PBVI_GEMM_NO_STREAMK")) : 0;
    pl.streamk = !single_chunk && !no_streamk;
    pl.nblocks = device_cu_count();
    if (single_chunk) {
        pl.chunk_len = pl.k_tiles;
        pl.max_chunks = 1;
    } else if (pl.streamk) {
        const int max_split = 8;
        pl.chunk_len = pl.k_tiles;
        pl.max_chunks = max_split + 1;
        pl.c_floats = pl.slab_stride + (int64_t)pl.nblocks * (256 * 256);
        return pl;
    } else {
        pl.chunk_len = choose_chunk_len(pl.tiles_m * pl.tiles_n, pl.k_tiles);
        pl.max_chunks = (pl.k_tiles + pl.chunk_len - 1) / pl.chunk_len;
    }
    pl.c_floats = (int64_t)pl.max_chunks * pl.slab_stride;
    return pl;
}

size_t streamk_workspace_ints(const GemmPlan& pl) {
    const size_t pairs = (size_t)pl.tiles_m * pl.tiles_n;
    return (pairs + 1) + (size_t)pl.nblocks + pairs + 2;
}

template <typename T>
__global__ void k_gemm_nt_simple(const T* __restrict__ A, int lda, const T* __restrict__ B, int ldb,
                                 T* __restrict__ C, int ldc, int M, int N, int K) {
    __shared__ T As[16][17];
    __shared__ T Bs[16][17];
    const int tx = threadIdx.x, ty = threadIdx.y;
    const int m = blockIdx.y * 16 + ty, n = blockIdx.x * 16 + tx;
    T acc = 0;
    for (int k0 = 0; k0 < K; k0 += 16) {
        const int ka = k0 + tx;
        const int ma = blockIdx.y * 16 + ty, nb = blockIdx.x * 16 + ty;
        As[ty][tx] = (ma < M && ka < K) ? A[(int64_t)ma * lda + ka] : T(0);
        Bs[ty][tx] = (nb < N && ka < K) ? B[(int64_t)nb * ldb + ka] : T(0);
        __syncthreads();
#pragma unroll
        for (int kk = 0; kk < 16; ++kk) acc += As[ty][kk] * Bs[tx][kk];
        __syncthreads();
    }
    if (m < M && n < N) C[(int64_t)m * ldc + n] = acc;
}

template <typename T>
hipError_t launch_gemm_nt_simple(const T* A, int lda, const T* B, int ldb, T* C, int ldc, int M, int N,
                                 int K, hipStream_t stream) {
    if (M <= 0 || N <= 0) return hipSuccess;
    dim3 grid((N + 15) / 16, (M + 15) / 16), block(16, 16);
    hipLaunchKernelGGL(k_gemm_nt_simple<T>, grid, block, 0, stream, A, lda, B, ldb, C, ldc, M, N, K);
    return hipGetLastError();
}

template hipError_t launch_gemm_nt_simple<float>(const float*, int, const float*, int, float*, int, int, int, int, hipStream_t);
template hipError_t launch_gemm_nt_simple<double>(const double*, int, const double*, int, double*, int, int, int, int, hipStream_t);

}
```

### pomdp_pbvi_exploration_amd/csrc/pbvi_common.h

```cpp
#pragma once
#include <hip/hip_runtime.h>
#include <stdint.h>
#include <string>

#include "../../include/pbvi_hip.h"

namespace pbvi {

void set_error(const std::string& msg);

constexpr int GEMM_BM = 256;
constexpr int GEMM_BN = 256;
constexpr int GEMM_BK = 32;

inline int64_t round_up(int64_t x, int64_t m) { return (x + m - 1) / m * m; }

struct GemmPlan {
    int tiles_m, tiles_n, k_tiles, chunk_len, max_chunks, ldc;
    int64_t slab_stride;
    bool streamk;
    int nblocks;
    int64_t c_floats;
};
int set_gemm_force_dense(int enable);
int gemm_force_dense();
size_t streamk_workspace_ints(const GemmPlan& pl);
struct FusedB {
    const float* alpha;
    int lda;
    const int32_t* rs;
    const float* rto;
    int S_pad, O, V;
    int R;
    float gamma;
    const int32_t* ctile;
    const uint8_t* mat;
    const int32_t* irr;
};
GemmPlan make_gemm_plan(int M_pad, int N_pad, int K_pad, bool single_chunk = false);
hipError_t launch_tile_nonzero_f32(const float* X, int ld, int rows_pad, int k_tiles, uint8_t* nz, hipStream_t stream);
hipError_t launch_gemm_nt_f32(const float* A, int lda, const float* B, int ldb, float* C, const GemmPlan& pl,
                              const uint8_t* nzA, const uint8_t* nzB, int G, int v_group, int n_rows, int* klist,
                              int* kcount, int* nchunks, hipStream_t stream, int batch = 1,
                              int64_t batch_stride_b = 0, int64_t batch_stride_c = 0, int* streamk_ws = nullptr,
                              hipStream_t list_stream = nullptr, hipEvent_t list_event = nullptr,
                              hipEvent_t ev_before = nullptr, hipEvent_t ev_after = nullptr,
                              const FusedB* fused = nullptr, int split = 0);
int gemm_split_supported(int device);
size_t gemm_f64_klist_ints(int M, int N, int kt32);
size_t gemm_f64_pairs(int M, int N);
int gemm_f64_bn(int N);
size_t gemm_f64_kcount_ints(int M, int N, int kt32);
hipError_t launch_tile_nonzero_f64(const double* X, int ld, int rows, int kt32, uint8_t* nz, hipStream_t stream);
hipError_t launch_gemm_nt_f64(const double* A, int lda, int M, const double* B, int ldb, int N, double* C, int ldc,
                              int K_pad, const uint8_t* nzA, const uint8_t* nzB, int G, int v_group, int* klist,
                              int* kcount, hipStream_t stream, int split = 1 ,
                              int64_t slab_stride = 0 );
int gemm_f64_split(int M, int N, int kt32);
hipError_t launch_gemm_nt_f64_bf32(const double* A, int lda, int M, const float* B, int ldb, int N, double* C, int ldc,
                                   int K_pad, const uint8_t* nzA, int* klist, int* kcount, hipStream_t stream, int split = 1,
                                   int64_t slab_stride = 0);
hipError_t launch_gemm_nt_f64_ff32(const float* A, int lda, int M, const float* B, int ldb, int N, double* C, int ldc, int K_pad,
                                   const uint8_t* nzA, int* klist, int* kcount, hipStream_t stream, int split = 1,
                                   int64_t slab_stride = 0);
template <typename T>
hipError_t launch_gemm_nt_simple(const T* A, int lda, const T* B, int ldb, T* C, int ldc,
                                 int M, int N, int K, hipStream_t stream);


}
```

### pomdp_pbvi_exploration_amd/engine.py

```python
from __future__ import annotations

import ctypes as C
import os
from dataclasses import dataclass

import numpy as np

PKG_DIR = os.path.dirname(os.path.abspath(__file__))
LIB_PATH = os.path.join(PKG_DIR, 'libpbvi_hip.so')

PBVI_F32, PBVI_F64 = 0, 1
PBVI_SPARSE, PBVI_DENSE = 0, 1
PBVI_BELIEF_DOMINANCE = 1

EXPORTS = [
    'pbvi_version', 'pbvi_device_count', 'pbvi_last_error', 'pbvi_engine_create', 'pbvi_engine_destroy',
    'pbvi_alpha_set', 'pbvi_alpha_append', 'pbvi_alpha_count', 'pbvi_beliefs_set', 'pbvi_backup_run',
    'pbvi_backup_fetch', 'pbvi_backup_unique_count', 'pbvi_backup_fetch_unique', 'pbvi_backup_device_results',
    'pbvi_backup', 'pbvi_prune_dominated', 'pbvi_value_max',
    'pbvi_set_tie_window', 'pbvi_device_bytes',
    'pbvi_alpha_store_append', 'pbvi_alpha_select', 'pbvi_alpha_store_reset',
    'pbvi_belief_store_append', 'pbvi_beliefs_select', 'pbvi_belief_store_reset', 'pbvi_debug_poison',
    'pbvi_belief_update', 'pbvi_beliefs_advance', 'pbvi_beliefs_fetch', 'pbvi_beliefs_count',
    'pbvi_mdp_value_iteration', 'pbvi_set_formulation', 'pbvi_belief_walk', 'pbvi_engine_set_rto_f64', 'pbvi_backup_fetch_unique_keys', 'pbvi_assemble_rows',
    'pbvi_backup_fetch_exchange', 'pbvi_backup_store_unique',
    'pbvi_value_max_store', 'pbvi_belief_store_count', 'pbvi_alpha_store_count', 'pbvi_set_value_max_exact', 'pbvi_alpha_layout',
    'pbvi_belief_walk_keys', 'pbvi_backup_fetch_value_max',
    'pbvi_backup_fetch_compact', 'pbvi_host_alloc', 'pbvi_host_free', 'pbvi_debug_gemm_dense',
    'pbvi_backup_fetch_exchange_padded', 'pbvi_assemble_rows_store', 'pbvi_exchange_merge', 'pbvi_backup_run_fetch', 'pbvi_debug_alloc_limit', 'pbvi_engine_after_oom', 'pbvi_set_f64_screen', 'pbvi_set_fused_projection', 'pbvi_backup_fetch_row_hashes', 'pbvi_set_score_split',
    'pbvi_set_gamma_tiling', 'pbvi_gamma_tiling_plan',
]


class EngineUnavailable(RuntimeError):
    """The HIP library is missing or no GPU is visible."""


class PbviStats(C.Structure):
    _fields_ = [('ms_total', C.c_double), ('ms_project', C.c_double), ('ms_score', C.c_double),
                ('ms_argmax', C.c_double), ('ms_refine', C.c_double), ('ms_action', C.c_double),
                ('ms_assemble', C.c_double), ('ms_dominance', C.c_double), ('n_pairs', C.c_int64),
                ('n_dead', C.c_int64), ('n_refined', C.c_int64), ('n_refined_actions', C.c_int64),
                ('n_unique', C.c_int64),
                ('score_flops', C.c_int64), ('score_flops_executed', C.c_int64), ('score_tiles_dense', C.c_int64),
                ('score_tiles_run', C.c_int64), ('project_flops', C.c_int64), ('project_flops_executed', C.c_int64),
                ('split_k', C.c_int32), ('formulation', C.c_int32), ('n_refine_candidates', C.c_int64),
                ('ms_project_gemm', C.c_double), ('screened', C.c_int32), ('fused_projection', C.c_int32),
                ('score_split', C.c_int32), ('gamma_chunks', C.c_int32)]

    def as_dict(self) -> dict:
        return {name: getattr(self, name) for name, _ in self._fields_}


_lib = None


def load_library(path: str = LIB_PATH):
    global _lib
    if _lib is not None:
        return _lib
    path = os.environ.get('PBVI_LIB_PATH', path)
    if not os.path.exists(path):
        raise EngineUnavailable(f'{path} not found: build it with `python -m pomdp_pbvi_exploration_amd.build`')
    try:
        lib = C.CDLL(path)
    except OSError as e:
        raise EngineUnavailable(f'cannot load {path}: {e}') from e
    vp, i32p, u8p, f64p = C.c_void_p, C.POINTER(C.c_int32), C.POINTER(C.c_uint8), C.POINTER(C.c_double)
    sp = C.POINTER(PbviStats)
    protos = {
        'pbvi_version': (C.c_int, []),
        'pbvi_device_count': (C.c_int, []),
        'pbvi_last_error': (C.c_char_p, []),
        'pbvi_engine_create': (C.c_int, [C.POINTER(vp), C.c_int, C.c_int32, C.c_int32, C.c_int32, C.c_int32,
                                         i32p, vp, vp, C.c_int, C.c_int]),
        'pbvi_engine_destroy': (None, [vp]),
        'pbvi_alpha_set': (C.c_int, [vp, vp, C.c_int64]),
        'pbvi_alpha_append': (C.c_int, [vp, vp, C.c_int64]),
        'pbvi_alpha_count': (C.c_int64, [vp]),
        'pbvi_beliefs_set': (C.c_int, [vp, vp, C.c_int64]),
        'pbvi_backup_run': (C.c_int, [vp, C.c_double, C.c_int, sp]),
        'pbvi_backup_fetch': (C.c_int, [vp, vp, i32p, i32p, u8p]),
        'pbvi_backup_unique_count': (C.c_int64, [vp]),
        'pbvi_backup_fetch_unique': (C.c_int, [vp, vp, i32p]),
        'pbvi_backup_fetch_compact': (C.c_int, [vp, vp, i32p, i32p, i32p, u8p]),
        'pbvi_host_alloc': (vp, [C.c_size_t]),
        'pbvi_host_free': (None, [vp]),
        'pbvi_debug_gemm_dense': (C.c_int, [C.c_int]),
        'pbvi_backup_store_unique': (C.c_int64, [vp, i32p, C.c_int64]),
        'pbvi_backup_device_results': (C.c_int, [vp, C.POINTER(vp), C.POINTER(vp), C.POINTER(vp)]),
        'pbvi_backup': (C.c_int, [vp, vp, C.c_int64, C.c_double, C.c_int, vp, i32p, i32p, u8p, sp]),
        'pbvi_prune_dominated': (C.c_int, [vp, u8p]),
        'pbvi_value_max': (C.c_int, [vp, f64p, i32p]),
        'pbvi_value_max_store': (C.c_int, [vp, C.c_int64, f64p, i32p]),
        'pbvi_belief_store_count': (C.c_int64, [vp]),
        'pbvi_backup_fetch_value_max': (C.c_int, [vp, f64p]),
        'pbvi_belief_walk_keys': (C.c_int, [vp, C.c_int64, C.POINTER(C.c_uint64)]),
        'pbvi_set_value_max_exact': (C.c_int, [vp, C.c_int]),
        'pbvi_alpha_layout': (C.c_int, [vp, C.POINTER(C.c_int64), C.POINTER(C.c_int64)]),
        'pbvi_alpha_store_count': (C.c_int64, [vp]),
        'pbvi_alpha_store_append': (C.c_int64, [vp, vp, C.c_int64]),
        'pbvi_alpha_select': (C.c_int, [vp, i32p, C.c_int64]),
        'pbvi_alpha_store_reset': (C.c_int, [vp]),
        'pbvi_belief_store_append': (C.c_int64, [vp, vp, C.c_int64]),
        'pbvi_beliefs_select': (C.c_int, [vp, i32p, C.c_int64]),
        'pbvi_belief_store_reset': (C.c_int, [vp]),
        'pbvi_debug_poison': (C.c_int, [C.c_int]),
        'pbvi_belief_update': (C.c_int, [vp, i32p, i32p, vp]),
        'pbvi_beliefs_advance': (C.c_int, [vp, i32p, i32p, u8p, C.POINTER(C.c_int64)]),
        'pbvi_beliefs_fetch': (C.c_int, [vp, vp]),
        'pbvi_beliefs_count': (C.c_int64, [vp]),
        'pbvi_mdp_value_iteration': (C.c_int, [C.c_int, C.c_int32, C.c_int32, C.c_int32, i32p, f64p, f64p, f64p,
                                               C.c_double, C.c_double, C.c_int32, f64p, f64p, i32p]),
        'pbvi_set_formulation': (C.c_int, [vp, C.c_int]),
        'pbvi_set_f64_screen': (C.c_int, [vp, C.c_int]),
        'pbvi_set_fused_projection': (C.c_int, [vp, C.c_int]),
        'pbvi_set_score_split': (C.c_int, [vp, C.c_int]),
        'pbvi_set_gamma_tiling': (C.c_int, [vp, C.c_int, C.c_int64]),
        'pbvi_gamma_tiling_plan': (C.c_int, [C.c_int32, C.c_int32, C.c_int32, C.c_int64, C.c_int64, C.c_int, C.c_int64,
                                            C.POINTER(C.c_int64), C.POINTER(C.c_int64), C.POINTER(C.c_int64)]),
        'pbvi_belief_walk': (C.c_int64, [vp, f64p, C.c_int64, i32p, i32p, u8p, f64p]),
        'pbvi_engine_set_rto_f64': (C.c_int, [vp, f64p]),
        'pbvi_backup_fetch_unique_keys': (C.c_int, [vp, vp]),
        'pbvi_backup_fetch_row_hashes': (C.c_int, [vp, C.POINTER(C.c_uint64)]),
        'pbvi_assemble_rows': (C.c_int, [vp, C.c_double, C.c_int64, vp, vp]),
        'pbvi_backup_fetch_exchange': (C.c_int, [vp, vp]),
        'pbvi_backup_fetch_exchange_padded': (C.c_int, [vp, C.c_int64, vp]),
        'pbvi_assemble_rows_store': (C.c_int64, [vp, C.c_double, C.c_int64, vp, vp]),
        'pbvi_backup_run_fetch': (C.c_int, [vp, C.c_double, C.c_int, sp, vp, C.c_int64, i32p, i32p, i32p, i32p, u8p,
                                           C.POINTER(C.c_int64), C.POINTER(C.c_int64)]),
        'pbvi_debug_alloc_limit': (C.c_int64, [C.c_int64]),
        'pbvi_engine_after_oom': (C.c_int, [vp]),
        'pbvi_exchange_merge': (C.c_int64, [vp, C.c_int32, C.c_int64, C.c_int64, C.c_int32, C.c_int64, vp, vp, vp, vp]),
        'pbvi_set_tie_window': (C.c_int, [vp, C.c_double]),
        'pbvi_device_bytes': (C.c_int64, [vp]),
    }
    for name, (res, args) in protos.items():
        fn = getattr(lib, name)
        fn.restype = res
        fn.argtypes = args
    _lib = lib
    return lib


def debug_poison(enable: bool) -> bool:
    return bool(load_library().pbvi_debug_poison(1 if enable else 0))


def debug_alloc_limit(mb: int) -> int:
    return int(load_library().pbvi_debug_alloc_limit(int(mb)))


def gamma_tiling_plan(S: int, A: int, O: int, V: int, B: int, dtype: str = 'f32', budget_bytes: int = 0,
                      chunk_rows: int = 0) -> tuple:
    if dtype not in ('f32', 'f64'):
        raise ValueError("dtype must be 'f32' or 'f64'")
    for name, v in (('S', S), ('A', A), ('O', O)):
        if not -2**31 <= int(v) < 2**31:
            raise ValueError(f'{name} out of range')
    rows, n, need = C.c_int64(int(chunk_rows)), C.c_int64(0), C.c_int64(0)
    _check(load_library().pbvi_gamma_tiling_plan(int(S), int(A), int(O), int(V), int(B), 0 if dtype == 'f32' else 1,
                                                 int(budget_bytes), C.byref(rows), C.byref(n), C.byref(need)))
    return int(rows.value), int(n.value), int(need.value)


def debug_gemm_dense(enable: bool) -> bool:
    return bool(load_library().pbvi_debug_gemm_dense(1 if enable else 0))


def device_count() -> int:
    return int(load_library().pbvi_device_count())


class _PinnedArray(np.ndarray):

    def __array_finalize__(self, obj):
        self._owner = getattr(obj, '_owner', None)


class PinnedBuffer:

    def __init__(self, nbytes: int):
        self._lib = load_library()
        self.nbytes = int(nbytes)
        self._p = self._lib.pbvi_host_alloc(self.nbytes)
        if not self._p:
            raise MemoryError((self._lib.pbvi_last_error() or b'').decode(errors='replace'))
        self._raw = (C.c_uint8 * self.nbytes).from_address(self._p)
        self._off = 0
        self._views = []

    def carve(self, shape, dtype) -> np.ndarray:
        dtype = np.dtype(dtype)
        n = int(np.prod(shape)) * dtype.itemsize
        off = (self._off + 255) // 256 * 256
        if off + n > self.nbytes:
            raise MemoryError('PinnedBuffer exhausted')
        self._off = off + n
        import weakref
        arr = np.frombuffer(self._raw, dtype=dtype, count=int(np.prod(shape)), offset=off).reshape(shape).view(_PinnedArray)
        arr._owner = self
        self._views.append(weakref.ref(arr))
        return arr

    def close(self) -> None:
        if getattr(self, '_p', None):
            if any(r() is not None for r in self._views):
                raise RuntimeError('PinnedBuffer.close(): arrays carved from it are still referenced')
            self._raw = None
            self._lib.pbvi_host_free(self._p)
            self._p = None

    def __del__(self):
        try:
            self.close()
        except Exception:
            pass


def mdp_value_iteration(reach_states: np.ndarray, reach_prob: np.ndarray, exp_reward: np.ndarray, v0: np.ndarray,
                        gamma: float, max_change_limit: float, horizon: int, device: int = 0):
    lib = load_library()
    S, A, R = reach_states.shape
    if int(reach_states.min()) < 0 or int(reach_states.max()) >= S:
        raise ValueError('reachable state out of range')
    rs = np.ascontiguousarray(reach_states, dtype=np.int32)
    p = np.ascontiguousarray(reach_prob, dtype=np.float64)
    er = np.ascontiguousarray(exp_reward, dtype=np.float64)
    v = np.ascontiguousarray(v0, dtype=np.float64)
    if p.shape != (S, A, R) or er.shape != (S, A) or v.shape != (S,):
        raise ValueError('mdp_value_iteration: table shapes do not agree')
    rows = np.empty((A, S), dtype=np.float64)
    changes = np.zeros(max(int(horizon), 1), dtype=np.float64)
    its = C.c_int32(0)
    f64p, i32p = C.POINTER(C.c_double), C.POINTER(C.c_int32)
    _check(lib.pbvi_mdp_value_iteration(int(device), S, A, R, rs.ctypes.data_as(i32p), p.ctypes.data_as(f64p),
                                        er.ctypes.data_as(f64p), v.ctypes.data_as(f64p), float(gamma),
                                        float(max_change_limit), int(horizon), rows.ctypes.data_as(f64p),
                                        changes.ctypes.data_as(f64p), C.byref(its)))
    return rows, changes[:its.value]


def _check(rc: int) -> None:
    if rc == 0:
        return
    msg = (load_library().pbvi_last_error() or b'').decode(errors='replace')
    if rc == -2:
        raise MemoryError(msg)
    if rc == -1:
        raise ValueError(msg)
    if rc == -4:
        raise NotImplementedError(msg)
    raise RuntimeError(f'pbvi engine error {rc}: {msg}')


def _ptr(a: np.ndarray):
    return a.ctypes.data_as(C.c_void_p)


class HostArena:

    BLOCK_BYTES = 1 << 30
    _MIN_BLOCK = 1 << 20
    _POPULATE_MIN = 32 << 20
    _POPULATE_CHUNK = 64 << 20
    _MADV_POPULATE_WRITE = 23

    def __init__(self, first_block_bytes: int = 0):
        self._block = None
        self._off = 0
        self._next = max(self._MIN_BLOCK, min(self.BLOCK_BYTES, 1 << max(0, int(first_block_bytes) - 1).bit_length()))

    @classmethod
    def _populate(cls, block: np.ndarray) -> None:
        import threading
        try:
            libc = C.CDLL(None, use_errno=True)
            madvise = libc.madvise
        except (OSError, AttributeError):
            return
        madvise.argtypes = [C.c_void_p, C.c_size_t, C.c_int]
        madvise.restype = C.c_int
        page = 4096
        lo = (block.ctypes.data + page - 1) // page * page
        hi = (block.ctypes.data + block.shape[0]) // page * page

        def work(keep_alive=block):
            a = lo
            while a < hi:
                n = min(cls._POPULATE_CHUNK, hi - a)
                if madvise(a, n, cls._MADV_POPULATE_WRITE) != 0:
                    return
                a += n
        threading.Thread(target=work, name='pbvi-arena-populate', daemon=True).start()

    def empty(self, shape, dtype) -> np.ndarray:
        dtype = np.dtype(dtype)
        n = int(np.prod(shape)) * dtype.itemsize
        if n == 0 or n > self.BLOCK_BYTES // 4:
            return np.empty(shape, dtype=dtype)
        off = (self._off + 63) // 64 * 64
        if self._block is None or off + n > self._block.shape[0]:
            size = self._next
            while size < 4 * n:
                size *= 2
            size = min(size, self.BLOCK_BYTES)
            self._next = min(size * 2, self.BLOCK_BYTES)
            self._block = np.empty(size, dtype=np.uint8)
            if size >= self._POPULATE_MIN:
                self._populate(self._block)
            off = 0
        self._off = off + n
        return self._block[off:off + n].view(dtype).reshape(shape)


@dataclass
class BackupResult:
    unique_alpha: np.ndarray
    index: np.ndarray
    actions: np.ndarray
    best_alpha_ind: np.ndarray
    keep: np.ndarray
    stats: dict

    @property
    def alpha(self) -> np.ndarray:
        return self.unique_alpha[self.index]

    def value_function_rows(self, use_keep: bool = False, with_index: bool = False):
        idx = self.index[self.keep] if use_keep else self.index
        act = self.actions[self.keep] if use_keep else self.actions
        if idx.size == 0:
            return (self.unique_alpha[:0], act[:0], idx[:0]) if with_index else (self.unique_alpha[:0], act[:0])
        first = np.unique(idx, return_index=True)[1]
        first.sort()
        sel = idx[first]
        whole = len(sel) == len(self.unique_alpha) and bool((sel == np.arange(len(sel))).all())
        rows = self.unique_alpha if whole else self.unique_alpha[sel]
        if with_index:
            return rows, act[first], sel
        return rows, act[first]


class Engine:

    _serials = iter(range(1, 1 << 62))
    _nonce = None

    def __init__(self, S: int, A: int, O: int, R: int, reach_states: np.ndarray, rto: np.ndarray,
                 exp_rewards: np.ndarray, dtype: str = 'f32', mode: str = 'sparse', device: int = 0):
        lib = load_library()
        if lib.pbvi_device_count() <= 0:
            raise EngineUnavailable('no HIP device visible to libpbvi_hip.so')
        assert dtype in ('f32', 'f64')
        self.dtype = dtype
        self.np_dtype = np.float32 if dtype == 'f32' else np.float64
        self.S, self.A, self.O, self.R = int(S), int(A), int(O), int(R)
        self.device = device
        rs = np.asarray(reach_states)
        assert rs.shape == (S, A, R), f'reachable_states must be [S,A,R]={S, A, R}, got {rs.shape}'
        if rs.size and (rs.min() < 0 or rs.max() >= S):
            raise ValueError('reachable_states entry out of range [0,S)')
        rs32 = np.ascontiguousarray(rs, dtype=np.int32)
        rto_c = np.ascontiguousarray(rto, dtype=self.np_dtype)
        er_c = np.ascontiguousarray(exp_rewards, dtype=self.np_dtype)
        assert rto_c.shape == (S, A, O, R) and er_c.shape == (S, A)
        self._h = C.c_void_p()
        _check(lib.pbvi_engine_create(C.byref(self._h), device, S, A, O, R,
                                      rs32.ctypes.data_as(C.POINTER(C.c_int32)), _ptr(rto_c), _ptr(er_c),
                                      PBVI_F32 if dtype == 'f32' else PBVI_F64,
                                      PBVI_SPARSE if mode == 'sparse' else PBVI_DENSE))
        self._lib = lib
        if Engine._nonce is None or Engine._nonce[0] != os.getpid():
            import secrets
            Engine._nonce = (os.getpid(), secrets.randbits(48))
        self.serial = Engine._nonce + (next(Engine._serials),)
        self._alpha_token = None
        self._formulation = None
        self._gamma_tiling = None
        self.last_stats = {}
        self._store_epoch = {'alpha': 0, 'belief': 0}
        self._resident = {'alpha': None, 'belief': None}
        self.B = 0
        self._vmax_cache, self._vmax_epochs = [], None
        self._arena = HostArena(first_block_bytes=128 * self.S * 8)
        if dtype == 'f32' and np.asarray(rto).dtype == np.float64:
            r64 = np.ascontiguousarray(rto, dtype=np.float64)
            self._ck(lib.pbvi_engine_set_rto_f64(self._h, r64.ctypes.data_as(C.POINTER(C.c_double))))

    @classmethod
    def for_model(cls, model, dtype: str = 'f64', device: int = 0, mode: str = 'sparse') -> 'Engine':
        return cls(model.state_count, model.action_count, model.observation_count, model.reachable_state_count,
                   model.reachable_states, model.reachable_transitional_observation_table,
                   model.expected_rewards_table, dtype=dtype, mode=mode, device=device)

    def close(self) -> None:
        if getattr(self, '_h', None) is not None and self._h:
            self._lib.pbvi_engine_destroy(self._h)
            self._h = None

    def __del__(self):
        try:
            self.close()
        except Exception:
            pass

    def _ck(self, rc: int) -> None:
        if rc == -2:
            msg = (self._lib.pbvi_last_error() or b'').decode(errors='replace')
            self._lib.pbvi_engine_after_oom(self._h)
            self._resident = {'alpha': None, 'belief': None}
            for k in self._store_epoch:
                self._store_epoch[k] += 1
            self._vmax_cache, self._vmax_epochs = [], None
            self._alpha_token = None
            self.B = 0
            raise MemoryError(msg)
        _check(rc)

    def _as_rows(self, arr: np.ndarray) -> np.ndarray:
        a = np.ascontiguousarray(arr, dtype=self.np_dtype)
        if a.ndim != 2 or a.shape[1] != self.S:
            raise ValueError(f'expected a [*, {self.S}] array, got {a.shape}')
        return a

    def set_alpha(self, alpha: np.ndarray) -> None:
        a = self._as_rows(alpha)
        self._resident['alpha'] = None
        self._ck(self._lib.pbvi_alpha_set(self._h, _ptr(a), a.shape[0]))
        self._alpha_token = None

    def append_alpha(self, alpha: np.ndarray) -> None:
        a = self._as_rows(alpha)
        self._resident['alpha'] = None
        self._ck(self._lib.pbvi_alpha_append(self._h, _ptr(a), a.shape[0]))
        self._alpha_token = None

    @property
    def alpha_count(self) -> int:
        return int(self._lib.pbvi_alpha_count(self._h))

    def set_beliefs(self, beliefs: np.ndarray) -> None:
        b = self._as_rows(beliefs)
        self._resident['belief'] = None
        self._ck(self._lib.pbvi_beliefs_set(self._h, _ptr(b), b.shape[0]))
        self.B = b.shape[0]

    def store_rows(self, which: str, rows: np.ndarray) -> int:
        a = self._as_rows(rows)
        fn = self._lib.pbvi_alpha_store_append if which == 'alpha' else self._lib.pbvi_belief_store_append
        first = int(fn(self._h, _ptr(a), a.shape[0]))
        if first < 0:
            self._ck(first)
        return first

    def store_unique(self, unique_idx) -> int:
        i = np.ascontiguousarray(unique_idx, dtype=np.int32)
        first = int(self._lib.pbvi_backup_store_unique(self._h, i.ctypes.data_as(C.POINTER(C.c_int32)), i.shape[0]))
        if first < 0:
            self._ck(first)
        return first

    def store_tag(self, which: str):
        return (self.serial, which, self._store_epoch[which])

    def select_alpha(self, ids) -> None:
# ... 462 lines not shown
```

Measured before the change: 652,900.

## Restructure stream-K plan with locality-aware pair order and whole-tile body blocks

```diff
diff --git a/include/pbvi_hip.h b/include/pbvi_hip.h
--- a/include/pbvi_hip.h
+++ b/include/pbvi_hip.h
@@ -158,6 +158,11 @@
 int pbvi_gamma_tiling_plan(int32_t S, int32_t A, int32_t O, int64_t V, int64_t B, int dtype, int64_t budget_bytes,
                            int64_t* chunk_rows, int64_t* n_chunks, int64_t* bytes_needed);
 
+int pbvi_streamk_plan(const int32_t* kcount, int32_t tiles_m, int32_t tiles_n, int32_t nblocks, int32_t k_tiles, int32_t ovh,
+                      int32_t order, int32_t groups, int32_t group_tiles, int32_t ranges, int32_t* first_block,
+                      int32_t* nchunks, int32_t* segs, int64_t seg_cap, int64_t* n_segs, int32_t* share);
+int pbvi_streamk_order(void);
+
 int pbvi_set_tie_window(pbvi_engine_t* e, double rel);
 
 int pbvi_debug_poison(int enable);
diff --git a/pomdp_pbvi_exploration_amd/csrc/engine.hip b/pomdp_pbvi_exploration_amd/csrc/engine.hip
--- a/pomdp_pbvi_exploration_amd/csrc/engine.hip
+++ b/pomdp_pbvi_exploration_amd/csrc/engine.hip
@@ -3849,6 +3849,24 @@
                               std::to_string(tp.bytes) + " bytes, the budget is " + std::to_string(budget_bytes));
     return PBVI_OK;
 }
+int pbvi_streamk_plan(const int32_t* kcount, int32_t tiles_m, int32_t tiles_n, int32_t nblocks, int32_t k_tiles, int32_t ovh,
+                      int32_t order, int32_t groups, int32_t group_tiles, int32_t ranges, int32_t* first_block,
+                      int32_t* nchunks, int32_t* segs, int64_t seg_cap, int64_t* n_segs, int32_t* share) {
+    using namespace pbvi;
+    if (!kcount || !first_block || !nchunks || !n_segs || !share || (seg_cap > 0 && !segs) || seg_cap < 0)
+        FAIL(PBVI_EINVAL, "streamk_plan: null argument");
+    if (tiles_m < 1 || tiles_n < 1 || (int64_t)tiles_m * tiles_n > 0x7fffffff || nblocks < 1 || k_tiles < 1 || ovh < 0 ||
+        (order != 0 && order != 1) || groups < 0 || group_tiles < 0 || ranges < 1 || ranges > 65536)
+        FAIL(PBVI_EINVAL, "streamk_plan: tiles_m, tiles_n, nblocks, k_tiles must be positive, ovh, groups, group_tiles >= 0, order 0 or 1, ranges in [1, 65536]");
+    const int64_t pairs = (int64_t)tiles_m * tiles_n;
+    for (int64_t p = 0; p < pairs; ++p)
+        if (kcount[p] < 0 || kcount[p] > k_tiles) FAIL(PBVI_EINVAL, "streamk_plan: a list length outside [0, k_tiles]");
+    const SkOrder ord = {order, tiles_m, tiles_n, groups, group_tiles};
+    if (streamk_plan_host(kcount, ord, nblocks, k_tiles, ovh, ranges, first_block, nchunks, segs, seg_cap, n_segs, share) != 0)
+        FAIL(PBVI_EINVAL, "streamk_plan: the lists' total cost exceeds int32");
+    return PBVI_OK;
+}
+int pbvi_streamk_order(void) { return pbvi::streamk_order_local(); }
 int pbvi_set_tie_window(pbvi_engine_t* e, double rel) {
     NEED(e);
     return e->impl->set_tie_window(rel);
diff --git a/pomdp_pbvi_exploration_amd/csrc/gemm.hip b/pomdp_pbvi_exploration_amd/csrc/gemm.hip
--- a/pomdp_pbvi_exploration_amd/csrc/gemm.hip
+++ b/pomdp_pbvi_exploration_amd/csrc/gemm.hip
@@ -1,9 +1,13 @@
 #include "pbvi_common.h"
 #include "split_bf16.h"
-
+#include "streamk_plan.h"
+
+#include <algorithm>
 #include <cstdlib>
+#include <cstring>
 #include <map>
 #include <mutex>
+#include <vector>
 
 namespace pbvi {
 
@@ -161,103 +165,95 @@
 }
 
 __global__ void k_streamk_plan(const int* __restrict__ kcount, int pairs, int nblocks, int k_tiles, int max_split,
-                               int ovh, int* __restrict__ prefix, int* __restrict__ start_pair,
+                               int ovh, SkOrder ord, int* __restrict__ tpre, int* __restrict__ start,
                                int* __restrict__ first_block, int* __restrict__ nchunks, int* __restrict__ plan) {
-    __shared__ int part[256];
-    __shared__ int q_sh;
+    __shared__ long long part_t[256];
+    __shared__ int part_b[256], part_c[256];
+    __shared__ int q_sh, nbody_sh;
     const int tid = threadIdx.x;
     const int per = (pairs + 255) / 256;
-    const int p0 = (tid * per < pairs) ? tid * per : pairs;
-    const int p1 = (p0 + per < pairs) ? p0 + per : pairs;
-    int sum = 0;
-    for (int p = p0; p < p1; ++p) {
-        const int cnt = kcount[p];
-        sum += cnt > 0 ? cnt + ovh : 0;
-    }
-    part[tid] = sum;
-    for (int i = tid; i < nblocks; i += 256) start_pair[i] = -1;
+    const int j0 = (tid * per < pairs) ? tid * per : pairs;
+    const int j1 = (j0 + per < pairs) ? j0 + per : pairs;
+    part_t[tid] = sk_range_cost(kcount, ord, j0, j1, ovh);
+    for (int i = tid; i < nblocks; i += 256) start[i] = -1;
+    __syncthreads();
+    if (tid == 0) {
+        long long run = 0;
+        for (int i = 0; i < 256; ++i) run += part_t[i];
+        const int q = sk_share(run, nblocks, k_tiles, ovh, max_split);
+        q_sh = q;
+        plan[0] = q;
+        plan[1] = (int)run;
+    }
+    __syncthreads();
+    const int q = q_sh;
+    {
+        int64_t tail;
+        int bodies;
+        sk_range_tail(kcount, ord, j0, j1, q, ovh, tail, bodies);
+        __syncthreads();
+        part_t[tid] = tail;
+        part_b[tid] = bodies;
+    }
+    __syncthreads();
+    if (tid == 0) {
+        long long run = 0;
+        int nb = 0;
+        for (int i = 0; i < 256; ++i) {
+            const long long v = part_t[i];
+            const int w = part_b[i];
+            part_t[i] = run;
+            part_b[i] = nb;
+            run += v;
+            nb += w;
+        }
+        nbody_sh = nb;
+        plan[2] = nb;
+        plan[3] = (int)run;
+        tpre[pairs] = (int)run;
+    }
+    __syncthreads();
+    part_c[tid] = sk_range_conts(kcount, ord, j0, j1, q, ovh, part_t[tid]);
     __syncthreads();
     if (tid == 0) {
         int run = 0;
         for (int i = 0; i < 256; ++i) {
-            const int v = part[i];
-            part[i] = run;
+            const int v = part_c[i];
+            part_c[i] = run;
             run += v;
         }
-        int q = (run + nblocks - 1) / nblocks;
-        const int qmin = (k_tiles + ovh + max_split - 1) / max_split;
-        if (q < qmin) q = qmin;
-        if (q < 1) q = 1;
-        q_sh = q;
-        plan[0] = q;
-        plan[1] = run;
-        prefix[pairs] = run;
     }
     __syncthreads();
-    const int q = q_sh;
-    int run = part[tid];
-    for (int p = p0; p < p1; ++p) {
-        const int cnt = kcount[p];
-        prefix[p] = run;
-        if (cnt > 0) {
-            const int cost = cnt + ovh;
-            const int fb = run / q, lb = (run + cost - 1) / q;
-            const int fw = (run + ovh) / q;
-            first_block[p] = fw;
-            nchunks[p] = lb - fw + 1;
-            for (int i = fb; i <= lb; ++i)
-                if ((int64_t)i * q >= run) start_pair[i] = p;
-            run += cost;
-        } else {
-            first_block[p] = 0;
-            nchunks[p] = 0;
-        }
-    }
+    sk_range_emit(kcount, ord, j0, j1, q, ovh, nblocks, nbody_sh, part_t[tid], part_b[tid], part_c[tid], tpre, start,
+                  first_block, nchunks);
+}
+
+__device__ __forceinline__ int streamk_logical_id() {
+    const int nb = gridDim.x;
+    const int bid = blockIdx.x, xcd = bid & 7, qq = nb >> 3, r = nb & 7;
+    const int base = (xcd < r) ? xcd * (qq + 1) : r * (qq + 1) + (xcd - r) * qq;
+    return base + (bid >> 3);
 }
 
 __global__ __launch_bounds__(512) void k_gemm_nt_f32_streamk(
     const float* __restrict__ A, int lda, const float* __restrict__ B, int ldb, float* __restrict__ C, int ldc,
     int64_t slab_stride, int tiles_m, int pairs, int k_tiles, const int* __restrict__ klist,
-    const int* __restrict__ kcount, const int* __restrict__ prefix, const int* __restrict__ start_pair,
-    const int* __restrict__ first_block, const int* __restrict__ plan, int ovh) {
+    SkView sk) {
     extern __shared__ __attribute__((aligned(16))) float lds[];
-    const int nb = gridDim.x;
-    int L;
-    {
-        const int bid = blockIdx.x, xcd = bid & 7, qq = nb >> 3, r = nb & 7;
-        const int base = (xcd < r) ? xcd * (qq + 1) : r * (qq + 1) + (xcd - r) * qq;
-        L = base + (bid >> 3);
-    }
-    const int q = plan[0], T = plan[1];
-    int64_t pos = (int64_t)L * q;
-    if (pos >= T) return;
-    const int64_t end = (pos + q < T) ? pos + q : T;
-    int p = start_pair[L];
-    if (p < 0) return;
+    SkCursor cur;
+    sk_begin(sk, streamk_logical_id(), cur);
     TileThread t;
     t.init();
-    while (pos < end && p < pairs) {
-        const int cnt = kcount[p];
-        if (cnt == 0) {
-            ++p;
-            continue;
-        }
-        const int u_lo = (int)(pos - prefix[p]);
-        const int64_t room = end - pos;
-        const int u_hi = (u_lo + room < cnt + ovh) ? (int)(u_lo + room) : cnt + ovh;
-        const int lo = u_lo > ovh ? u_lo - ovh : 0;
-        const int hi = u_hi > ovh ? u_hi - ovh : 0;
-        if (hi > lo) {
-            const int tm = p % tiles_m, tn = p / tiles_m;
-            f32x16 acc[4][2];
-            tile_zero(acc);
-            tile_run(t, lds, A + (int64_t)tm * 256 * lda, lda, B + (int64_t)tn * 256 * ldb, ldb,
-                     klist + (int64_t)p * k_tiles, lo, hi, acc);
-            const bool cont = L != first_block[p];
-            tile_store(t, cont ? C + slab_stride + (int64_t)L * (256 * 256) : C, cont ? 256 : ldc, cont ? 0 : tm, cont ? 0 : tn, acc);
-        }
-        pos += u_hi - u_lo;
-        ++p;
+    SkSeg seg;
+    while (sk_next(sk, cur, seg)) {
+        const int p = seg.pair, lo = seg.lo, hi = seg.hi;
+        const int tm = p % tiles_m, tn = p / tiles_m;
+        f32x16 acc[4][2];
+        tile_zero(acc);
+        tile_run(t, lds, A + (int64_t)tm * 256 * lda, lda, B + (int64_t)tn * 256 * ldb, ldb,
+                 klist + (int64_t)p * k_tiles, lo, hi, acc);
+        const bool cont = seg.slot != 0;
+        tile_store(t, cont ? C + slab_stride + (int64_t)seg.slot * (256 * 256) : C, cont ? 256 : ldc, cont ? 0 : tm, cont ? 0 : tn, acc);
     }
 }
 
@@ -373,57 +369,32 @@
 
 __global__ __launch_bounds__(512) void k_gemm_nt_f32_streamk_fused(
     const float* __restrict__ A, int lda, const float* __restrict__ B, int ldb, FusedB fb, float* __restrict__ C, int ldc,
-    int64_t slab_stride, int tiles_m, int pairs, int k_tiles, const int* __restrict__ klist, const int* __restrict__ kcount,
-    const int* __restrict__ prefix, const int* __restrict__ start_pair, const int* __restrict__ first_block,
-    const int* __restrict__ plan, int ovh) {
+    int64_t slab_stride, int tiles_m, int pairs, int k_tiles, const int* __restrict__ klist, SkView sk) {
     extern __shared__ __attribute__((aligned(16))) float lds[];
-    const int nb = gridDim.x;
-    int L;
-    {
-        const int bid = blockIdx.x, xcd = bid & 7, qq = nb >> 3, r = nb & 7;
-        const int base = (xcd < r) ? xcd * (qq + 1) : r * (qq + 1) + (xcd - r) * qq;
-        L = base + (bid >> 3);
-    }
-    const int q = plan[0], T = plan[1];
-    int64_t pos = (int64_t)L * q;
-    if (pos >= T) return;
-    const int64_t end = (pos + q < T) ? pos + q : T;
-    int p = start_pair[L];
-    if (p < 0) return;
+    SkCursor cur;
+    sk_begin(sk, streamk_logical_id(), cur);
     TileThread t;
     t.init();
-    while (pos < end && p < pairs) {
-        const int cnt = kcount[p];
-        if (cnt == 0) {
-            ++p;
-            continue;
-        }
-        const int u_lo = (int)(pos - prefix[p]);
-        const int64_t room = end - pos;
-        const int u_hi = (u_lo + room < cnt + ovh) ? (int)(u_lo + room) : cnt + ovh;
-        const int lo = u_lo > ovh ? u_lo - ovh : 0;
-        const int hi = u_hi > ovh ? u_hi - ovh : 0;
-        if (hi > lo) {
-            const int tm = p % tiles_m, tn = p / tiles_m;
-            f32x16 acc[4][2];
-            tile_zero(acc);
-            if (fb.mat[tn]) {
-                const int bt = fb.ctile != nullptr ? fb.ctile[tn] : tn;
-                tile_run(t, lds, A + (int64_t)tm * 256 * lda, lda, B + (int64_t)bt * 256 * ldb, ldb,
-                         klist + (int64_t)p * k_tiles, lo, hi, acc);
-            } else {
-                const int r0 = tn * 256;
-                const int g = r0 / fb.V, v0 = r0 - g * fb.V;
-                tile_run_fused(t, lds, A + (int64_t)tm * 256 * lda, lda, fb.rs + (int64_t)(g / fb.O) * fb.S_pad,
-                               fb.rto + (int64_t)g * fb.S_pad, fb.alpha + (int64_t)(v0 + t.srow[0]) * fb.lda,
-                               (int64_t)64 * fb.lda, fb.gamma,
-                               klist + (int64_t)p * k_tiles, lo, hi, acc);
-            }
-            const bool cont = L != first_block[p];
-            tile_store(t, cont ? C + slab_stride + (int64_t)L * (256 * 256) : C, cont ? 256 : ldc, cont ? 0 : tm, cont ? 0 : tn, acc);
-        }
-        pos += u_hi - u_lo;
-        ++p;
+    SkSeg seg;
+    while (sk_next(sk, cur, seg)) {
+        const int p = seg.pair, lo = seg.lo, hi = seg.hi;
+        const int tm = p % tiles_m, tn = p / tiles_m;
+        f32x16 acc[4][2];
+        tile_zero(acc);
+        if (fb.mat[tn]) {
+            const int bt = fb.ctile != nullptr ? fb.ctile[tn] : tn;
+            tile_run(t, lds, A + (int64_t)tm * 256 * lda, lda, B + (int64_t)bt * 256 * ldb, ldb,
+                     klist + (int64_t)p * k_tiles, lo, hi, acc);
+        } else {
+            const int r0 = tn * 256;
+            const int g = r0 / fb.V, v0 = r0 - g * fb.V;
+            tile_run_fused(t, lds, A + (int64_t)tm * 256 * lda, lda, fb.rs + (int64_t)(g / fb.O) * fb.S_pad,
+                           fb.rto + (int64_t)g * fb.S_pad, fb.alpha + (int64_t)(v0 + t.srow[0]) * fb.lda,
+                           (int64_t)64 * fb.lda, fb.gamma,
+                           klist + (int64_t)p * k_tiles, lo, hi, acc);
+        }
+        const bool cont = seg.slot != 0;
+        tile_store(t, cont ? C + slab_stride + (int64_t)seg.slot * (256 * 256) : C, cont ? 256 : ldc, cont ? 0 : tm, cont ? 0 : tn, acc);
     }
 }
 
@@ -588,56 +559,31 @@
 template <int R>
 __global__ __launch_bounds__(512) void k_gemm_nt_f32_streamk_fused_r(
     const float* __restrict__ A, int lda, const float* __restrict__ B, int ldb, FusedB fb, float* __restrict__ C, int ldc,
-    int64_t slab_stride, int tiles_m, int pairs, int k_tiles, const int* __restrict__ klist, const int* __restrict__ kcount,
-    const int* __restrict__ prefix, const int* __restrict__ start_pair, const int* __restrict__ first_block,
-    const int* __restrict__ plan, int ovh) {
+    int64_t slab_stride, int tiles_m, int pairs, int k_tiles, const int* __restrict__ klist, SkView sk) {
     extern __shared__ __attribute__((aligned(16))) float lds[];
-    const int nb = gridDim.x;
-    int L;
-    {
-        const int bid = blockIdx.x, xcd = bid & 7, qq = nb >> 3, r = nb & 7;
-        const int base = (xcd < r) ? xcd * (qq + 1) : r * (qq + 1) + (xcd - r) * qq;
-        L = base + (bid >> 3);
-    }
-    const int q = plan[0], T = plan[1];
-    int64_t pos = (int64_t)L * q;
-    if (pos >= T) return;
-    const int64_t end = (pos + q < T) ? pos + q : T;
-    int p = start_pair[L];
-    if (p < 0) return;
+    SkCursor cur;
+    sk_begin(sk, streamk_logical_id(), cur);
     TileThread t;
     t.init();
-    while (pos < end && p < pairs) {
-        const int cnt = kcount[p];
-        if (cnt == 0) {
-            ++p;
-            continue;
-        }
-        const int u_lo = (int)(pos - prefix[p]);
-        const int64_t room = end - pos;
-        const int u_hi = (u_lo + room < cnt + ovh) ? (int)(u_lo + room) : cnt + ovh;
-        const int lo = u_lo > ovh ? u_lo - ovh : 0;
-        const int hi = u_hi > ovh ? u_hi - ovh : 0;
-        if (hi > lo) {
-            const int tm = p % tiles_m, tn = p / tiles_m;
-            f32x16 acc[4][2];
-            tile_zero(acc);
-            if (fb.mat[tn]) {
-                tile_run(t, lds, A + (int64_t)tm * 256 * lda, lda, B + (int64_t)tn * 256 * ldb, ldb,
-                         klist + (int64_t)p * k_tiles, lo, hi, acc);
-            } else {
-                const int r0 = tn * 256;
-                const int g = r0 / fb.V, v0 = r0 - g * fb.V;
-                tile_run_fused_r<R>(t, lds, A + (int64_t)tm * 256 * lda, lda, B + (int64_t)tn * 256 * ldb, ldb,
-                                 fb.rs + (int64_t)(g / fb.O) * R * fb.S_pad, fb.rto + (int64_t)g * R * fb.S_pad,
-                                 fb.S_pad, fb.alpha + (int64_t)(v0 + t.srow[0]) * fb.lda, (int64_t)64 * fb.lda, fb.gamma,
-                                 klist + (int64_t)p * k_tiles, lo, hi, acc);
-            }
-            const bool cont = L != first_block[p];
-            tile_store(t, cont ? C + slab_stride + (int64_t)L * (256 * 256) : C, cont ? 256 : ldc, cont ? 0 : tm, cont ? 0 : tn, acc);
-        }
-        pos += u_hi - u_lo;
-        ++p;
+    SkSeg seg;
+    while (sk_next(sk, cur, seg)) {
+        const int p = seg.pair, lo = seg.lo, hi = seg.hi;
+        const int tm = p % tiles_m, tn = p / tiles_m;
+        f32x16 acc[4][2];
+        tile_zero(acc);
+        if (fb.mat[tn]) {
+            tile_run(t, lds, A + (int64_t)tm * 256 * lda, lda, B + (int64_t)tn * 256 * ldb, ldb,
+                     klist + (int64_t)p * k_tiles, lo, hi, acc);
+        } else {
+            const int r0 = tn * 256;
+            const int g = r0 / fb.V, v0 = r0 - g * fb.V;
+            tile_run_fused_r<R>(t, lds, A + (int64_t)tm * 256 * lda, lda, B + (int64_t)tn * 256 * ldb, ldb,
+                             fb.rs + (int64_t)(g / fb.O) * R * fb.S_pad, fb.rto + (int64_t)g * R * fb.S_pad,
+                             fb.S_pad, fb.alpha + (int64_t)(v0 + t.srow[0]) * fb.lda, (int64_t)64 * fb.lda, fb.gamma,
+                             klist + (int64_t)p * k_tiles, lo, hi, acc);
+        }
+        const bool cont = seg.slot != 0;
+        tile_store(t, cont ? C + slab_stride + (int64_t)seg.slot * (256 * 256) : C, cont ? 256 : ldc, cont ? 0 : tm, cont ? 0 : tn, acc);
     }
 }
 
@@ -821,57 +767,32 @@
 
 __global__ __launch_bounds__(512) void k_gemm_split_streamk(
     const float* __restrict__ A, int lda, const float* __restrict__ B, int ldb, FusedB fb, float* __restrict__ C, int ldc,
-    int64_t slab_stride, int tiles_m, int pairs, int k_tiles, const int* __restrict__ klist, const int* __restrict__ kcount,
-    const int* __restrict__ prefix, const int* __restrict__ start_pair, const int* __restrict__ first_block,
-    const int* __restrict__ plan, int ovh) {
+    int64_t slab_stride, int tiles_m, int pairs, int k_tiles, const int* __restrict__ klist, SkView sk) {
     extern __shared__ __attribute__((aligned(16))) float lds[];
-    const int nb = gridDim.x;
-    int L;
-    {
-        const int bid = blockIdx.x, xcd = bid & 7, qq = nb >> 3, r = nb & 7;
-        const int base = (xcd < r) ? xcd * (qq + 1) : r * (qq + 1) + (xcd - r) * qq;
-        L = base + (bid >> 3);
-    }
-    const int q = plan[0], T = plan[1];
-    int64_t pos = (int64_t)L * q;
-    if (pos >= T) return;
-    const int64_t end = (pos + q < T) ? pos + q : T;
-    int p = start_pair[L];
-    if (p < 0) return;
+    SkCursor cur;
+    sk_begin(sk, streamk_logical_id(), cur);
     TileThread t;
     t.init();
-    while (pos < end && p < pairs) {
-        const int cnt = kcount[p];
-        if (cnt == 0) {
-            ++p;
-            continue;
-        }
-        const int u_lo = (int)(pos - prefix[p]);
-        const int64_t room = end - pos;
-        const int u_hi = (u_lo + room < cnt + ovh) ? (int)(u_lo + room) : cnt + ovh;
-        const int lo = u_lo > ovh ? u_lo - ovh : 0;
-        const int hi = u_hi > ovh ? u_hi - ovh : 0;
-        if (hi > lo) {
-            const int tm = p % tiles_m, tn = p / tiles_m;
-            f32x16 acc[4][2];
-            tile_zero(acc);
-            const float* Ablk = A + (int64_t)tm * 256 * lda;
-            if (fb.mat == nullptr || fb.mat[tn]) {
-                const int bt = (fb.mat != nullptr && fb.ctile != nullptr) ? fb.ctile[tn] : tn;
-                tile_run_split(t, lds, Ablk, lda, B + (int64_t)bt * 256 * ldb, ldb, false, nullptr, nullptr, nullptr, 0, 0.f,
-                               klist + (int64_t)p * k_tiles, lo, hi, acc);
-            } else {
-                const int r0 = tn * 256;
-                const int g = r0 / fb.V, v0 = r0 - g * fb.V;
-                tile_run_split(t, lds, Ablk, lda, nullptr, 0, true, fb.rs + (int64_t)(g / fb.O) * fb.S_pad,
-                               fb.rto + (int64_t)g * fb.S_pad, fb.alpha + (int64_t)(v0 + (threadIdx.x >> 2)) * fb.lda,
-                               (int64_t)128 * fb.lda, fb.gamma, klist + (int64_t)p * k_tiles, lo, hi, acc);
-            }
-            const bool cont = L != first_block[p];
-            tile_store(t, cont ? C + slab_stride + (int64_t)L * (256 * 256) : C, cont ? 256 : ldc, cont ? 0 : tm, cont ? 0 : tn, acc);
-        }
-        pos += u_hi - u_lo;
-        ++p;
+    SkSeg seg;
+    while (sk_next(sk, cur, seg)) {
+        const int p = seg.pair, lo = seg.lo, hi = seg.hi;
+        const int tm = p % tiles_m, tn = p / tiles_m;
+        f32x16 acc[4][2];
+        tile_zero(acc);
+        const float* Ablk = A + (int64_t)tm * 256 * lda;
+        if (fb.mat == nullptr || fb.mat[tn]) {
+            const int bt = (fb.mat != nullptr && fb.ctile != nullptr) ? fb.ctile[tn] : tn;
+            tile_run_split(t, lds, Ablk, lda, B + (int64_t)bt * 256 * ldb, ldb, false, nullptr, nullptr, nullptr, 0, 0.f,
+                           klist + (int64_t)p * k_tiles, lo, hi, acc);
+        } else {
+            const int r0 = tn * 256;
+            const int g = r0 / fb.V, v0 = r0 - g * fb.V;
+            tile_run_split(t, lds, Ablk, lda, nullptr, 0, true, fb.rs + (int64_t)(g / fb.O) * fb.S_pad,
+                           fb.rto + (int64_t)g * fb.S_pad, fb.alpha + (int64_t)(v0 + (threadIdx.x >> 2)) * fb.lda,
+                           (int64_t)128 * fb.lda, fb.gamma, klist + (int64_t)p * k_tiles, lo, hi, acc);
+        }
+        const bool cont = seg.slot != 0;
+        tile_store(t, cont ? C + slab_stride + (int64_t)seg.slot * (256 * 256) : C, cont ? 256 : ldc, cont ? 0 : tm, cont ? 0 : tn, acc);
     }
 }
 
@@ -1027,6 +948,75 @@
     return (int)len;
 }
 
+int streamk_order_local() {
+    static const int local = [] {
+        const char* env = getenv("PBVI_STREAMK_ORDER");
+        return (env != nullptr && strcmp(env, "local") == 0) ? 1 : 0;
+    }();
+    return local;
+}
+
+int streamk_plan_host(const int* kcount, const SkOrder& ord, int nblocks, int k_tiles, int ovh, int ranges, int* first_block,
+                      int* nchunks, int* segs, int64_t seg_cap, int64_t* n_segs, int* q_out) {
+    const int pairs = ord.tiles_m * ord.tiles_n;
+    std::vector<int> tpre((size_t)pairs + 1), start((size_t)nblocks, -1);
+    std::vector<int64_t> part_t((size_t)ranges);
+    std::vector<int> part_b((size_t)ranges), part_c((size_t)ranges);
+    int plan[STREAMK_PLAN_INTS];
+    const int per = (pairs + ranges - 1) / ranges;
+    auto j0 = [&](int r) { return (int)std::min<int64_t>((int64_t)r * per, pairs); };
+    auto j1 = [&](int r) { return (int)std::min<int64_t>((int64_t)j0(r) + per, pairs); };
+    int64_t total = 0;
+    for (int r = 0; r < ranges; ++r) total += sk_range_cost(kcount, ord, j0(r), j1(r), ovh);
+    if (total > 0x7fffffff) return -1;
+    const int q = sk_share(total, nblocks, k_tiles, ovh, STREAMK_MAX_SPLIT);
+    int64_t tail = 0;
+    int bodies = 0;
+    for (int r = 0; r < ranges; ++r) {
+        int64_t t;
+        int b;
+        sk_range_tail(kcount, ord, j0(r), j1(r), q, ovh, t, b);
+        part_t[r] = tail;
+        part_b[r] = bodies;
+        tail += t;
+        bodies += b;
+    }
+    plan[0] = q;
+    plan[1] = (int)total;
+    plan[2] = bodies;
+    plan[3] = (int)tail;
+    tpre[pairs] = (int)tail;
+    int conts = 0;
+    for (int r = 0; r < ranges; ++r) {
+        part_c[r] = conts;
+        conts += sk_range_conts(kcount, ord, j0(r), j1(r), q, ovh, part_t[r]);
+    }
+    for (int r = 0; r < ranges; ++r)
+        sk_range_emit(kcount, ord, j0(r), j1(r), q, ovh, nblocks, bodies, part_t[r], part_b[r], part_c[r], tpre.data(),
+                      start.data(), first_block, nchunks);
+    const SkView sk = {kcount, tpre.data(), start.data(), first_block, plan, pairs, ovh, ord};
+    int64_t n = 0;
+    for (int L = 0; L < nblocks; ++L) {
+        SkCursor cur;
+        sk_begin(sk, L, cur);
+        SkSeg seg;
+        while (sk_next(sk, cur, seg)) {
+            if (n < seg_cap) {
+                int* o = segs + n * 5;
+                o[0] = L;
+                o[1] = seg.pair;
+                o[2] = seg.lo;
+                o[3] = seg.hi;
+                o[4] = seg.slot;
+            }
+            ++n;
+        }
+    }
+    *n_segs = n;
+    *q_out = q;
+    return 0;
+}
+
 static int device_cu_count() {
     static int cus = 0;
     if (cus == 0) {
@@ -1089,32 +1079,38 @@
     if (e != hipSuccess) return e;
     if (pl.streamk) {
         if (batch != 1 || streamk_ws == nullptr) return hipErrorInvalidValue;
-        int* prefix = streamk_ws;
-        int* start_pair = prefix + pairs + 1;
-        int* first_block = start_pair + pl.nblocks;
+        int* tpre = streamk_ws;
+        int* start = tpre + pairs + 1;
+        int* first_block = start + pl.nblocks;
         int* plan = first_block + pairs;
-        static const int ovh = getenv("PBVI_STREAMK_OVH") ? atoi(getenv("PBVI_STREAMK_OVH")) : 1;
+        static const int ovh = getenv("PBVI_STREAMK_OVH") ? std::max(0, atoi(getenv("PBVI_STREAMK_OVH"))) : 1;
+        SkOrder ord;
+        ord.local = streamk_order_local();
+        ord.tiles_m = pl.tiles_m;
+        ord.tiles_n = pl.tiles_n;
+        const bool grouped = nzB != nullptr && G > 0 && v_group > 0 && v_group % GEMM_BN == 0;
+        ord.groups = grouped ? G : 0;
+        ord.group_tiles = grouped ? v_group / GEMM_BN : 0;
         hipLaunchKernelGGL(k_streamk_plan, dim3(1), dim3(256), 0, ls, kcount, pairs, pl.nblocks, pl.k_tiles,
-                           pl.max_chunks - 1, ovh, prefix, start_pair, first_block, nchunks, plan);
+                           pl.max_chunks - 1, ovh, ord, tpre, start, first_block, nchunks, plan);
         e = hipGetLastError();
         if (e != hipSuccess) return e;
         if (ls != stream) {
             if ((e = hipEventRecord(list_event, ls)) != hipSuccess) return e;
             if ((e = hipStreamWaitEvent(stream, list_event, 0)) != hipSuccess) return e;
         }
+        const SkView sk = {kcount, tpre, start, first_block, plan, pairs, ovh, ord};
         if (split) {
             FusedB fb{};
             if (fused != nullptr) fb = *fused;
             hipLaunchKernelGGL(k_gemm_split_streamk, dim3(pl.nblocks), dim3(512), GEMM_LDS_BYTES, stream, A, lda, B, ldb, fb, C,
-                               pl.ldc, pl.slab_stride, pl.tiles_m, pairs, pl.k_tiles, klist, kcount, prefix, start_pair,
-                               first_block, plan, ovh);
+                               pl.ldc, pl.slab_stride, pl.tiles_m, pairs, pl.k_tiles, klist, sk);
         } else if (fused != nullptr && fused->R > 1) {
             switch (fused->R) {
 #define PBVI_FUSED_R_CASE(RR)                                                                                                   \
     case RR:                                                                                                                    \
         hipLaunchKernelGGL(k_gemm_nt_f32_streamk_fused_r<RR>, dim3(pl.nblocks), dim3(512), GEMM_LDS_BYTES_R, stream, A, lda, B, \
-                           ldb, *fused, C, pl.ldc, pl.slab_stride, pl.tiles_m, pairs, pl.k_tiles, klist, kcount, prefix,        \
-                           start_pair, first_block, plan, ovh);                                                                 \
+                           ldb, *fused, C, pl.ldc, pl.slab_stride, pl.tiles_m, pairs, pl.k_tiles, klist, sk);                   \
         break;
                 PBVI_FUSED_R_CASE(2) PBVI_FUSED_R_CASE(3) PBVI_FUSED_R_CASE(4) PBVI_FUSED_R_CASE(5) PBVI_FUSED_R_CASE(6) PBVI_FUSED_R_CASE(7)
 #undef PBVI_FUSED_R_CASE
@@ -1123,12 +1119,10 @@
             }
         } else if (fused != nullptr)
             hipLaunchKernelGGL(k_gemm_nt_f32_streamk_fused, dim3(pl.nblocks), dim3(512), GEMM_LDS_BYTES, stream, A, lda, B, ldb,
-                               *fused, C, pl.ldc, pl.slab_stride, pl.tiles_m, pairs, pl.k_tiles, klist, kcount, prefix, start_pair,
-                               first_block, plan, ovh);
+                               *fused, C, pl.ldc, pl.slab_stride, pl.tiles_m, pairs, pl.k_tiles, klist, sk);
         else
             hipLaunchKernelGGL(k_gemm_nt_f32_streamk, dim3(pl.nblocks), dim3(512), GEMM_LDS_BYTES, stream, A, lda, B, ldb, C,
-                               pl.ldc, pl.slab_stride, pl.tiles_m, pairs, pl.k_tiles, klist, kcount, prefix, start_pair,
-                               first_block, plan, ovh);
+                               pl.ldc, pl.slab_stride, pl.tiles_m, pairs, pl.k_tiles, klist, sk);
         return hipGetLastError();
     }
     if (ls != stream) {
@@ -1161,7 +1155,7 @@
         pl.chunk_len = pl.k_tiles;
         pl.max_chunks = 1;
     } else if (pl.streamk) {
-        const int max_split = 8;
+        const int max_split = STREAMK_MAX_SPLIT;
         pl.chunk_len = pl.k_tiles;
         pl.max_chunks = max_split + 1;
         pl.c_floats = pl.slab_stride + (int64_t)pl.nblocks * (256 * 256);
@@ -1176,7 +1170,7 @@
 
 size_t streamk_workspace_ints(const GemmPlan& pl) {
     const size_t pairs = (size_t)pl.tiles_m * pl.tiles_n;
-    return (pairs + 1) + (size_t)pl.nblocks + pairs + 2;
+    return (pairs + 1) + (size_t)pl.nblocks + pairs + STREAMK_PLAN_INTS;
 }
 
 template <typename T>
diff --git a/pomdp_pbvi_exploration_amd/csrc/pbvi_common.h b/pomdp_pbvi_exploration_amd/csrc/pbvi_common.h
--- a/pomdp_pbvi_exploration_amd/csrc/pbvi_common.h
+++ b/pomdp_pbvi_exploration_amd/csrc/pbvi_common.h
@@ -4,6 +4,7 @@
 #include <string>
 
 #include "../../include/pbvi_hip.h"
+#include "streamk_plan.h"
 
 namespace pbvi {
 
@@ -25,6 +26,9 @@
 int set_gemm_force_dense(int enable);
 int gemm_force_dense();
 size_t streamk_workspace_ints(const GemmPlan& pl);
+int streamk_plan_host(const int* kcount, const SkOrder& ord, int nblocks, int k_tiles, int ovh, int ranges, int* first_block,
+                      int* nchunks, int* segs, int64_t seg_cap, int64_t* n_segs, int* q_out);
+int streamk_order_local();
 struct FusedB {
     const float* alpha;
     int lda;
diff --git a/pomdp_pbvi_exploration_amd/csrc/streamk_plan.h b/pomdp_pbvi_exploration_amd/csrc/streamk_plan.h
--- /dev/null
+++ b/pomdp_pbvi_exploration_amd/csrc/streamk_plan.h
@@ -0,0 +1,188 @@
+#pragma once
+#include <stdint.h>
+
+#if defined(__HIPCC__)
+#define PBVI_SK_HD __host__ __device__ inline
+#else
+#define PBVI_SK_HD inline
+#endif
+
+namespace pbvi {
+
+constexpr int STREAMK_MAX_SPLIT = 8;
+constexpr int STREAMK_PLAN_INTS = 4;
+
+struct SkOrder {
+    int local;
+    int tiles_m, tiles_n;
+    int groups, group_tiles;
+};
+
+PBVI_SK_HD int sk_pair_at(const SkOrder& o, int j) {
+    if (!o.local) return j;
+    const int tm = j / o.tiles_n, r = j - tm * o.tiles_n;
+    int tn = r;
+    if (o.group_tiles > 1 && o.groups > 0 && r < o.groups * o.group_tiles && o.groups * o.group_tiles <= o.tiles_n) {
+        const int vb = r / o.groups, g = r - vb * o.groups;
+        tn = g * o.group_tiles + vb;
+    }
+    return tn * o.tiles_m + tm;
+}
+
+PBVI_SK_HD int sk_share(int64_t total, int nblocks, int k_tiles, int ovh, int max_split) {
+    int64_t q = (total + nblocks - 1) / nblocks;
+    const int qmin = (k_tiles + ovh + max_split - 1) / max_split;
+    if (q < qmin) q = qmin;
+    if (q < 1) q = 1;
+    return (int)q;
+}
+
+struct SkPair {
+    int cost;
+    int body;
+    int tail;
+};
+PBVI_SK_HD SkPair sk_pair(int cnt, int q, int ovh, int local) {
+    SkPair s;
+    s.cost = cnt > 0 ? cnt + ovh : 0;
+    s.body = (local && s.cost >= q && q > ovh) ? 1 : 0;
+    s.tail = s.cost - (s.body ? q : 0);
+    return s;
+}
+PBVI_SK_HD void sk_pair_segs(const SkPair& s, int64_t t0, int q, int ovh, int& tb_first, int& nseg) {
+    tb_first = 0;
+    nseg = 0;
+    if (s.cost == 0) return;
+    if (s.body) {
+        tb_first = (int)(t0 / q);
+        nseg = 1 + (s.tail > 0 ? (int)((t0 + s.tail - 1) / q) - tb_first + 1 : 0);
+    } else {
+        tb_first = (int)((t0 + ovh) / q);
+        nseg = (int)((t0 + s.tail - 1) / q) - tb_first + 1;
+    }
+}
+
+PBVI_SK_HD int64_t sk_range_cost(const int* kcount, const SkOrder& o, int j0, int j1, int ovh) {
+    int64_t sum = 0;
+    for (int j = j0; j < j1; ++j) {
+        const int cnt = kcount[sk_pair_at(o, j)];
+        sum += cnt > 0 ? cnt + ovh : 0;
+    }
+    return sum;
+}
+PBVI_SK_HD void sk_range_tail(const int* kcount, const SkOrder& o, int j0, int j1, int q, int ovh, int64_t& tail, int& bodies) {
+    tail = 0;
+    bodies = 0;
+    for (int j = j0; j < j1; ++j) {
+        const SkPair s = sk_pair(kcount[sk_pair_at(o, j)], q, ovh, o.local);
+        tail += s.tail;
+        bodies += s.body;
+    }
+}
+PBVI_SK_HD int sk_range_conts(const int* kcount, const SkOrder& o, int j0, int j1, int q, int ovh, int64_t t) {
+    int conts = 0;
+    for (int j = j0; j < j1; ++j) {
+        const SkPair s = sk_pair(kcount[sk_pair_at(o, j)], q, ovh, o.local);
+        int tbf, n;
+        sk_pair_segs(s, t, q, ovh, tbf, n);
+        if (n > 1) conts += n - 1;
+        t += s.tail;
+    }
+    return conts;
+}
+PBVI_SK_HD void sk_range_emit(const int* kcount, const SkOrder& o, int j0, int j1, int q, int ovh, int nblocks, int nbody,
+                              int64_t t, int b, int c, int* tpre, int* start, int* first_block, int* nchunks) {
+    for (int j = j0; j < j1; ++j) {
+        const int p = sk_pair_at(o, j);
+        const SkPair s = sk_pair(kcount[p], q, ovh, o.local);
+        int tbf, n;
+        sk_pair_segs(s, t, q, ovh, tbf, n);
+        tpre[j] = (int)t;
+        nchunks[p] = n;
+        first_block[p] = n > 1 ? c : 0;
+        if (n > 1) c += n - 1;
+        if (s.body) start[b++] = j;
+        if (s.tail > 0) {
+            const int64_t fb = t / q, lb = (t + s.tail - 1) / q;
+            for (int64_t i = fb; i <= lb; ++i)
+                if (i * q >= t && nbody + i < nblocks) start[nbody + i] = j;
+        }
+        t += s.tail;
+    }
+}
+
+struct SkView {
+    const int* kcount;
+    const int* tpre;
+    const int* start;
+    const int* first_block;
+    const int* plan;
+    int pairs, ovh;
+    SkOrder ord;
+};
+struct SkSeg {
+    int pair, lo, hi;
+    int slot;
+};
+struct SkCursor {
+    int j, q, body;
+    int64_t pos, end;
+};
+PBVI_SK_HD void sk_begin(const SkView& v, int L, SkCursor& c) {
+    c.q = v.plan[0];
+    const int nbody = v.plan[2];
+    const int64_t ttail = v.plan[3];
+    c.j = v.start[L];
+    c.body = 0;
+    c.pos = 0;
+    c.end = 0;
+    if (c.j < 0) return;
+    if (L < nbody) {
+        c.body = 1;
+        return;
+    }
+    c.pos = (int64_t)(L - nbody) * c.q;
+    if (c.pos >= ttail) return;
+    c.end = c.pos + c.q < ttail ? c.pos + c.q : ttail;
+}
+PBVI_SK_HD bool sk_next(const SkView& v, SkCursor& c, SkSeg& out) {
+    if (c.body) {
+        c.body = 0;
+        out.pair = sk_pair_at(v.ord, c.j);
+        out.lo = 0;
+        out.hi = c.q - v.ovh;
+        out.slot = 0;
+        return true;
+    }
+    while (c.pos < c.end && c.j < v.pairs) {
+        const int p = sk_pair_at(v.ord, c.j);
+        const SkPair s = sk_pair(v.kcount[p], c.q, v.ovh, v.ord.local);
+        if (s.tail == 0) {
+            ++c.j;
+            continue;
+        }
+        const int64_t t0 = v.tpre[c.j];
+        const int u_lo = (int)(c.pos - t0);
+        const int64_t room = c.end - c.pos;
+        const int u_hi = (u_lo + room < s.tail) ? (int)(u_lo + room) : s.tail;
+        const int base = s.body ? c.q : 0;
+        const int lo = base + u_lo > v.ovh ? base + u_lo - v.ovh : 0;
+        const int hi = base + u_hi > v.ovh ? base + u_hi - v.ovh : 0;
+        const int tb = (int)(c.pos / c.q);
+        c.pos += u_hi - u_lo;
+        ++c.j;
+        if (hi > lo) {
+            int tbf, n;
+            sk_pair_segs(s, t0, c.q, v.ovh, tbf, n);
+            const int z = s.body + tb - tbf;
+            out.pair = p;
+            out.lo = lo;
+            out.hi = hi;
+            out.slot = z == 0 ? 0 : v.first_block[p] + z;
+            return true;
+        }
+    }
+    return false;
+}
+
+}
diff --git a/pomdp_pbvi_exploration_amd/engine.py b/pomdp_pbvi_exploration_amd/engine.py
--- a/pomdp_pbvi_exploration_amd/engine.py
+++ b/pomdp_pbvi_exploration_amd/engine.py
@@ -28,7 +28,7 @@
     'pbvi_belief_walk_keys', 'pbvi_backup_fetch_value_max',
     'pbvi_backup_fetch_compact', 'pbvi_host_alloc', 'pbvi_host_free', 'pbvi_debug_gemm_dense',
     'pbvi_backup_fetch_exchange_padded', 'pbvi_assemble_rows_store', 'pbvi_exchange_merge', 'pbvi_backup_run_fetch', 'pbvi_debug_alloc_limit', 'pbvi_engine_after_oom', 'pbvi_set_f64_screen', 'pbvi_set_fused_projection', 'pbvi_backup_fetch_row_hashes', 'pbvi_set_score_split',
-    'pbvi_set_gamma_tiling', 'pbvi_gamma_tiling_plan',
+    'pbvi_set_gamma_tiling', 'pbvi_gamma_tiling_plan', 'pbvi_streamk_plan', 'pbvi_streamk_order',
 ]
 
 
@@ -119,6 +119,9 @@
         'pbvi_set_gamma_tiling': (C.c_int, [vp, C.c_int, C.c_int64]),
         'pbvi_gamma_tiling_plan': (C.c_int, [C.c_int32, C.c_int32, C.c_int32, C.c_int64, C.c_int64, C.c_int, C.c_int64,
                                             C.POINTER(C.c_int64), C.POINTER(C.c_int64), C.POINTER(C.c_int64)]),
+        'pbvi_streamk_plan': (C.c_int, [i32p, C.c_int32, C.c_int32, C.c_int32, C.c_int32, C.c_int32, C.c_int32, C.c_int32,
+                                        C.c_int32, C.c_int32, i32p, i32p, i32p, C.c_int64, C.POINTER(C.c_int64), i32p]),
+        'pbvi_streamk_order': (C.c_int, []),
         'pbvi_belief_walk': (C.c_int64, [vp, f64p, C.c_int64, i32p, i32p, u8p, f64p]),
         'pbvi_engine_set_rto_f64': (C.c_int, [vp, f64p]),
         'pbvi_backup_fetch_unique_keys': (C.c_int, [vp, vp]),
@@ -162,6 +165,34 @@
     _check(load_library().pbvi_gamma_tiling_plan(int(S), int(A), int(O), int(V), int(B), 0 if dtype == 'f32' else 1,
                                                  int(budget_bytes), C.byref(rows), C.byref(n), C.byref(need)))
     return int(rows.value), int(n.value), int(need.value)
+
+
+def streamk_order() -> str:
+    return 'local' if load_library().pbvi_streamk_order() else 'legacy'
+
+
+def streamk_plan(kcount, tiles_m: int, nblocks: int, k_tiles: int, ovh: int = 1, order: str = 'local', groups: int = 0,
+                 group_tiles: int = 0, ranges: int = 256) -> dict:
+    if order not in ('legacy', 'local'):
+        raise ValueError("order must be 'legacy' or 'local'")
+    kc = np.ascontiguousarray(kcount, dtype=np.int32).reshape(-1)
+    if tiles_m < 1 or kc.size == 0 or kc.size % tiles_m:
+        raise ValueError('kcount must hold tiles_n x tiles_m lengths')
+    tiles_n = kc.size // tiles_m
+    fb, nch = np.zeros(kc.size, np.int32), np.zeros(kc.size, np.int32)
+    n, share = C.c_int64(0), C.c_int32(0)
+    i32p = C.POINTER(C.c_int32)
+    cap = kc.size + int(nblocks) + 1
+    while True:
+        segs = np.zeros((cap, 5), np.int32)
+        _check(load_library().pbvi_streamk_plan(kc.ctypes.data_as(i32p), int(tiles_m), tiles_n, int(nblocks), int(k_tiles),
+                                                int(ovh), 1 if order == 'local' else 0, int(groups), int(group_tiles), int(ranges),
+                                                fb.ctypes.data_as(i32p), nch.ctypes.data_as(i32p), segs.ctypes.data_as(i32p),
+                                                cap, C.byref(n), C.byref(share)))
+        if n.value <= cap:
+            break
+        cap = int(n.value)
+    return {'share': int(share.value), 'first_block': fb, 'nchunks': nch, 'segs': segs[:n.value].copy()}
 
 
 def debug_gemm_dense(enable: bool) -> bool:
```

After: 641,500. -1.8%, worse.
